# navigator8972/vae_assoc

Hardware: AMD Instinct MI355X
Metric: paired-samples/sec (img+jnt assoc-VAE train step) (higher is better)
Workload: dtype bf16

## Files before the change

__graft_entry__.py:

```python
import os
import subprocess
import sys

ROOT = os.path.dirname(os.path.abspath(__file__))
CSRC = os.path.join(ROOT, "vae_assoc_amd", "csrc")
LIB = os.path.join(ROOT, "vae_assoc_amd", "libavae.so")
SOURCES = ["avae_kernels.hip", "avae_comm.hip", "avae_retrieve.hip", "avae_latent_stats.hip", "avae_aggpost.hip", "avae_gmm.hip", "avae_embed.hip", "avae_host.hip"]


FLAGS = ["--offload-arch=gfx950", "-O3", "-std=c++17", "-fPIC", "-shared", "-Wno-unused-result"]


def _source_hash():
    import hashlib
    h = hashlib.sha256(" ".join(FLAGS).encode())
    for path in sorted(os.path.join(CSRC, f) for f in os.listdir(CSRC)) + [os.path.join(ROOT, "include", "avae.h")]:
        h.update(os.path.basename(path).encode())
        with open(path, "rb") as f:
            h.update(f.read())
    return h.hexdigest()


def _stale(want):
    if not os.path.exists(LIB) or not os.path.exists(LIB + ".hash"):
        return True
    with open(LIB + ".hash") as f:
        return f.read().strip() != want


def build(force=False):
    import fcntl
    want = _source_hash()
    try:
        lock = open(LIB + ".lock", "w")
    except OSError:
        lock = None
        if force or _stale(want):
            raise
    if lock is not None:
        fcntl.flock(lock, fcntl.LOCK_EX)
        try:
            if force or _stale(want):
                hipcc = os.environ.get("HIPCC", "/opt/rocm/bin/hipcc")
                if not os.path.exists(hipcc):
                    hipcc = "hipcc"
                tmp = "%s.tmp.%d" % (LIB, os.getpid())
                cmd = [hipcc] + FLAGS + [os.path.join(CSRC, s) for s in SOURCES] + ["-o", tmp]
                subprocess.run(cmd, check=True, cwd=ROOT)
                os.replace(tmp, LIB)
                with open(LIB + ".hash", "w") as f:
                    f.write(want + "\n")
        finally:
            fcntl.flock(lock, fcntl.LOCK_UN)
            lock.close()
    if ROOT not in sys.path:
        sys.path.insert(0, ROOT)
    import vae_assoc_amd
    from vae_assoc_amd import _capi
    _capi.lib()


def smoke():
    if ROOT not in sys.path:
        sys.path.insert(0, ROOT)
    build()
    import numpy as np
    import torch
    from oracle import vae_assoc_oracle as O
    from vae_assoc_amd.vae_assoc import AssocVariationalAutoEncoder

    assert torch.cuda.is_available(), "smoke() needs the MI355X"
    img = dict(scope='image', hidden_conv=False, n_hidden_recog_1=96, n_hidden_recog_2=80,
               n_hidden_gener_1=96, n_hidden_gener_2=80, n_input=784, n_z=20)
    jnt = dict(scope='joint', hidden_conv=False, n_hidden_recog_1=72, n_hidden_recog_2=40,
               n_hidden_gener_1=72, n_hidden_gener_2=40, n_input=147, n_z=20)
    archs, B = [img, jnt], 48
    rng = np.random.default_rng(7)
    X = [rng.random((B, 784)).astype(np.float32), rng.standard_normal((B, 147)).astype(np.float32)]
    eps = rng.standard_normal((B, 20)).astype(np.float32)
    for dtype, tol in (("fp32", 2e-5), ("bf16", 2e-3)):
        model = AssocVariationalAutoEncoder(archs, binary=[True, False], transfer_fct="relu", weights=[50, 1],
                                            assoc_lambda=8.0, learning_rate=1e-3, batch_size=B,
                                            compute_dtype=dtype, device=0, seed=3)
        ref = O.OracleAssocVAE(archs, binary=[True, False], transfer_fct="relu", weights=[50, 1], assoc_lambda=8.0,
                               learning_rate=1e-3, batch_size=B, params_flat=model.get_params().astype(np.float64))
        c_hip = model.partial_fit(X, eps)
        c_ref = ref.partial_fit(X, eps)
        rel = abs(c_hip - c_ref) / abs(c_ref)
        assert rel < tol, "smoke: %s cost %.6f vs oracle %.6f (rel %.2e)" % (dtype, c_hip, c_ref, rel)
        dp = np.abs(model.get_params() - ref.get_params()).max()
        assert dp < 2.5e-3, "smoke: %s params drifted %.3e after one Adam step" % (dtype, dp)
        print("smoke %s: cost %.5f (oracle %.5f, rel %.2e), max|dtheta| %.2e" % (dtype, c_hip, c_ref, rel, dp))


if __name__ == "__main__":
    build(force="--force" in sys.argv)
    if "--smoke" in sys.argv:
        smoke()
```

vae_assoc_amd/csrc/avae_device.h:

```cpp
#pragma once
#include <hip/hip_runtime.h>
#include <math.h>
#include <stdint.h>
#include "../../include/avae.h"

namespace avae {

constexpr int kMaxMod = 4;
constexpr int kThreads = 256;
constexpr int kTileBytesK = 128;
constexpr int kRowAlign = 256;
constexpr int kLatentRows = 16;
constexpr int kAdamRows = 16;
constexpr int kCostHist = 4096;
constexpr int kSumsqThreads = 256;
constexpr int kSumsqMaxBlocks = 256;
constexpr int kSumsqQuads = 8;
inline int sumsq_blocks(long long p_int) {
    const long long quads = p_int / 4, per_block = (long long)kSumsqThreads * kSumsqQuads;
    const long long g = (quads + per_block - 1) / per_block;
    return (int)(g < 1 ? 1 : g > kSumsqMaxBlocks ? kSumsqMaxBlocks : g);
}
inline int sumsq_chain(long long p_int) {
    const long long quads = p_int / 4, per_pass = (long long)kSumsqThreads * sumsq_blocks(p_int);
    return (int)((quads + per_pass - 1) / per_pass);
}

enum Kind : int {
    K_FWD_HIDDEN = 0,
    K_FWD_HEAD = 1,
    K_FWD_OUT_LOSS = 2,
    K_FWD_OUT_STORE = 3,
    K_DGRAD_HIDDEN = 4,
    K_DGRAD_LATENT = 5,
    K_WGRAD = 6,
    K_DGRAD_F32 = 10,
    K_LATENT = 7,
    K_COST = 8,
    K_SERVE_Z = 11,
};

struct WorkItem {
    int kind;
    int M, N, K;
    int lda, ldb;
    int tiles_m, tiles_n;
    int act;
    int ld0, ld1, ldx;
    int nz;
    int binary;
    int ksplit, kchunk;
    int bias_row;
    int bias_ep;
    int kin;
    int tile_off, tile_cnt;
    int slot_base;
    int n_slots;
    int n_mod;
    int bump_step;
    float scale;
    float lambda;
    float inv_bg;
    const void* A;
    const void* B;
    void* out0;
    void* out1;
    void* out2;
    const void* aux0;
    const void* aux1;
    const void* aux2;
    float* partial;
    const float* eps;
    float wts[kMaxMod];
    const void* tail_w;
    void* tail_out;
    const void* tail_aux;
    int tail_mode;
    int tail_n;
    int tail_ldw, tail_ldo, tail_ldx;
    int tail_act;
    int tail_kt;
    int conv;
    const unsigned char* present;
    int present_ld;
};

struct ConvA {
    const void* src;
    const void* consts;
    int M, K;
    int OHW, OW, IH, IW, Cin;
    int k, so, d, pad;
    int src_sb, src_sp;
    int ones;
    unsigned mg_ohw, mg_ow, mg_k, mg_cin;
};
constexpr int kMaxConvA = 12;
constexpr int kMaxItemsPerLaunch = 12;
constexpr int kMaxPf = 4;
struct LaunchArgs {
    int n_items;
    int grid_x;
    int sched;
    int n_pf;
    const void* pf_ptr[4];
    int pf_lines[4];
    const ConvA* conv_tab;
    WorkItem items[kMaxItemsPerLaunch];
};

struct TnItem {
    const void* A;
    const void* B;
    float* out;
    int M, N, K;
    int lda, ldb, ld0;
    int tiles_m, tiles_n;
    int ksplit, kchunk;
    int bias_row;
    int tile_off, tile_cnt;
    int conv;
    void* W; void* Wt;
    int ldw, ldt;
};
constexpr int kMaxTnItems = 32;
constexpr int kTnPieces = 8;
struct TnPiece { unsigned short item, tile_off, cum_end, pad; };
struct DevState;
struct TnLaunchArgs {
    int n_items;
    int grid_x;
    int xcd_group;
    int sched;
    int adam;
    long long d_theta, d_m, d_v;
    float beta1, beta2, eps;
    const DevState* st;
    const ConvA* conv_tab;
    int xcd_pieces;
    TnPiece pieces[8][kTnPieces];
    TnItem items[kMaxTnItems];
};
static_assert(sizeof(TnLaunchArgs) <= 4096, "kernel arguments are passed by value: 4 KiB");

struct DevState {
    long long step;
    float last_cost;
    float lr_t;
    float cost_hist[kCostHist];
};

struct ClipState {
    float max_norm;
    int skip_nonfinite;
    long long n_skipped;
    float partial[kSumsqMaxBlocks];
    float norm_hist[kCostHist];
};

struct EmaState {
    float decay;
    int warmup;
    int pad[30];
};
static_assert(sizeof(EmaState) == 128, "the average is line-aligned behind its settings");

struct HyperEntry { float kl, lambda, lr, pad; };
constexpr int kHyperSets = 16;
struct SchedState {
    avae_schedule sched[3];
    float lambda0, lr0;
    HyperEntry tab[kHyperSets];
    float hist[kCostHist][3];
};

__host__ __device__ inline float schedule_value(const avae_schedule& s, long long t) {
#pragma clang fp contract(off)
    long long u = t - 1;
    if (u < 0) u = 0;
    if (s.kind == AVAE_SCHED_PIECEWISE) {
        if (s.period > 0) u %= s.period;
        const int last = s.n_knots - 1;
        if (u <= s.knot_step[0]) return s.knot_value[0];
        if (u >= s.knot_step[last]) return s.knot_value[last];
        int i = 0;
        while (i + 1 < last && u >= s.knot_step[i + 1]) ++i;
        const double v0 = (double)s.knot_value[i], v1 = (double)s.knot_value[i + 1];
        const double f = (double)(u - s.knot_step[i]) / (double)(s.knot_step[i + 1] - s.knot_step[i]);
        return (float)(v0 + (v1 - v0) * f);
    }
    if (s.kind == AVAE_SCHED_EXP) {
        const double e = s.staircase ? (double)(u / s.decay_steps) : (double)u / (double)s.decay_steps;
        return (float)pow((double)s.decay_rate, e);
    }
    return 1.0f;
}

struct AdamItem {
    float* theta;
    float* m;
    float* v;
    const float* g;
    void* W;
    void* Wt;
    int rows, cols;
    int ld, ldt;
    int tiles_r, tiles_c, tile_base;
    int ldw;
    void* Wadj; void* Wf;
    int ldadj, ldf, adj_k, adj_cin;
};

constexpr int kMaxAdamItems = 80;
struct AdamArgs {
    const AdamItem* items;
    int n_items;
    int base[kMaxAdamItems];
    int mode;
    int book;
    float lr, beta1, beta2, eps;
    DevState* st;
    const float* cost_src;
    ClipState* clip;
    int n_partial;
    const EmaState* ema;
    float* avg;
    const float* theta0;
};

struct PrepSeg {
    const float* src; int src_ld;
    int rows, cols;
    float* dst32; int ld32;
    void* dstc; int ldc;
    int tiles_r, tiles_c, tile_base;
    const float* src_in; int in_ld;
    unsigned drop_thr;
    float drop_value, noise_std;
};
struct PrepArgs {
    PrepSeg seg[kMaxMod];
    int n_seg;
    int total_tiles;
    const float* eps_src;
    float* eps_dst;
    int eps_rows, nz, eps_blocks, eps_ld;
    int row_offset;
    unsigned long long seed;
    const DevState* st;
    unsigned long long stream_salt;
    int n_steps, blocks_per_step;
    long long set_stride;
    const unsigned char* pres_src;
    unsigned char* pres_dst;
    int pres_ld;
    int noisy;
    SchedState* sched;
};

struct ReduceSeg { float* dst; const float* src; int n, parts; long long stride; int block_base;
                   int dst_ld;
                   int colsum;
                   int perm_k, perm_cin, perm_cout, perm_ldga, perm_ld; };
constexpr int kMaxReduceSegs = 40;
struct ReduceArgs { ReduceSeg seg[kMaxReduceSegs]; int n_seg; };

struct ConvGeom {
    int B, IH, IW, Cin, OH, OW, k, so, d, pad;
    int src_sb, src_sp;
    int ones;
};
struct GatherSeg {
    ConvGeom g;
    const void* src;
    void* P; int ldp;
    int tiles_r, tiles_c, tile_base;
    int cl, rpt;
};
struct GatherArgs { GatherSeg seg[kMaxMod]; int n_seg; };
struct Col2imSeg {
    ConvGeom g;
    const float* dP; int lddp;
    const void* yprev; int ldy;
    int act;
    void* dA; int lda;
    const float* g0; int nz;
    const void* bias; int bias_ld;
    int tiles_r, tiles_c, tile_base;
    int cl, rpt;
};
struct Col2imArgs { Col2imSeg seg[kMaxMod]; int n_seg; };

constexpr int kThinIn = 4096, kThinOut = 1024, kThinF = 1024;
constexpr int kThinSplit = 4;
struct ThinSeg {
    ConvGeom g;
    const void* X;
// ... 21 lines not shown
void launch_wadj(int compute_dtype, const WadjArgs& a, int n_blocks, hipStream_t s);
struct GpermSeg { const float* Gadj; float* G; int ldga, ld, k, Cin, Cout, block_base; };
struct GpermArgs { GpermSeg seg[2 * kMaxMod]; int n_seg; };
void launch_gperm(const GpermArgs& a, int n_blocks, hipStream_t s);
struct RowsumSeg { const void* src; float* part; int ld, rows, cols, cols4, cpow, n_blocks, block_base; };
struct RowsumArgs { RowsumSeg seg[2 * kMaxMod]; int n_seg; };
void launch_rowsum(int compute_dtype, const RowsumArgs& a, int n_blocks, hipStream_t s);

struct ServeSlot {
    const float* z;
    float* out[kMaxMod];
    int rows;
    int pad;
};
struct ServeArgs {
    ServeSlot* slot;
    int n_mod, nz, bucket;
    void* Z[kMaxMod]; int ldz[kMaxMod];
    int blocks_per_mod;
};
void launch_serve(int compute_dtype, const ServeArgs& a, const ServeSlot& call, int n_blocks, hipStream_t s);
struct ServeInMod { const void* w; void* out; int n, ldw, ldo, kt, act, slices; };
struct ServeInArgs {
    ServeSlot call;
    ServeSlot* slot;
    int n_mod, nz, bucket, tiles_m;
    ServeInMod mod[kMaxMod];
};
void launch_serve_in(int compute_dtype, const ServeInArgs& a, int grid_x, hipStream_t s);

void launch_gather(int compute_dtype, const GatherArgs& a, int n_blocks, hipStream_t s);
void launch_col2im(int compute_dtype, const Col2imArgs& a, int n_blocks, hipStream_t s);

constexpr int kScoreRows = kThreads / 64;
struct ScoreLatentArgs {
    const float* mulv[kMaxMod];
    void* Z[kMaxMod]; int ldz[kMaxMod];
    const float* eps; int ld_eps;
    float* out; int k;
    int rows, nz, n_mod;
    int src;
    const unsigned char* present;
};
void launch_score_latent(int compute_dtype, const ScoreLatentArgs& a, hipStream_t s);
struct ScoreRowsArgs {
    const float* xhat; int ld32;
    const float* x; long long ldx;
    float* out; int k;
    int rows, n_in, binary, col;
    int cost;
    int n_mod, n_pair;
    float w[kMaxMod]; float lambda;
    const unsigned char* present; int pa, pb; unsigned absent_bits;
};
void launch_score_rows(const ScoreRowsArgs& a, hipStream_t s);

struct IwLatentArgs {
    const float* mulv;
    const float* eps;
    float* z32;
    void* Z[kMaxMod]; int ldz[kMaxMod]; int n_zdst;
    float* r;
    int rows, kc, k0, K, nz;
    long long row0;
    unsigned long long seed; unsigned draw;
    const unsigned char* present; int pres_ld;
};
void launch_iw_latent(int compute_dtype, const IwLatentArgs& a, hipStream_t s);
struct IwRowsArgs {
    const float* xhat[kMaxMod]; int ldh[kMaxMod];
    const float* x[kMaxMod]; long long ldx[kMaxMod];
    int n_in[kMaxMod], binary[kMaxMod];
    float* ell;
    int n_dec, kc, n_mod;
    const unsigned char* present;
};
void launch_iw_rows(const IwRowsArgs& a, hipStream_t s);
struct IwReduceArgs {
    const float* ell; const float* r;
    float* state;
    float* out; int width;
    int rows, kc, src, n_mod;
    int first, last;
    float log_k;
    const unsigned char* present;
};
void launch_iw_reduce(const IwReduceArgs& a, hipStream_t s);

struct ImputeFuseArgs {
    const float* mulv[kMaxMod];
    unsigned mods;
    const unsigned char* present;
    float* fused;
    float* mu; float* lv;
    float* z32;
    void* Z[kMaxMod]; int ldz[kMaxMod]; int n_zdst;
    int rows, nz, n_mod;
};
void launch_impute_fuse(int compute_dtype, const ImputeFuseArgs& a, hipStream_t s);
struct ImputeAccumArgs {
    const float* xhat[kMaxMod]; int ldh[kMaxMod];
    float* mean[kMaxMod]; float* var[kMaxMod];
    int n_in[kMaxMod];
    int tile0[kMaxMod + 1];
    int col0[kMaxMod];
    float* state; int ld_state;
    int rows, kc, k0, K, n_mod;
};
void launch_impute_accum(const ImputeAccumArgs& a, hipStream_t s);

constexpr int kMaxWorld = 8;
constexpr int kIpcThreads = 256;
struct IpcArgs {
    float* g;
    long long off, granules;
    long long cost_idx;
    int world, rank, wire_bf16, blocks;
    unsigned char* peer[kMaxWorld];
    long long off_flag1, off_flag2;
    long long off_cost;
    long long off_seq;
    long long off_err;
    long long off_slots, slot_stride, off_res;
    unsigned long long timeout_ticks;
};
void launch_ipc_allreduce(const IpcArgs& a, hipStream_t s);
void launch_wire_pack(const float* g, void* wire, long long n, hipStream_t s);
void launch_wire_unpack(float* g, const void* wire, long long n, hipStream_t s);

struct LaunchEvents { hipEvent_t start, stop; };
extern thread_local LaunchEvents t_launch_events;

constexpr int kStampLaunches = 32, kStampBlocks = 1024, kStampWords = 8;

int tile_lds_bytes(int tile_cfg, bool two_c_tiles);
void launch_grouped(int compute_dtype, int tile_cfg, const LaunchArgs& args, int grid_x, int grid_y, int lds_bytes,
                    DevState* st, hipStream_t s, unsigned long long* stamps = nullptr, int launch_id = 0);
void launch_grouped_tn(int compute_dtype, int tile_cfg, const TnLaunchArgs& args, int grid_x, int grid_y, int lds_bytes,
                       DevState* st, hipStream_t s, unsigned long long* stamps = nullptr, int launch_id = 0);
void launch_adam(int compute_dtype, const AdamArgs& a, int n_blocks, hipStream_t s);
void launch_grad_sumsq(const float* g, long long p_int, float* partial, hipStream_t s);
void launch_prep(int compute_dtype, const PrepArgs& a, hipStream_t s);
const void* prep_kernel(int compute_dtype, bool masked, bool noisy, bool sched);
void launch_fill(void* base, int elem_bytes, unsigned bits, long long start, long long stride, int count, hipStream_t s);
void launch_sums(const ReduceArgs& a, int n_blocks, hipStream_t s);
int small_head_lds_bytes();
void launch_small_latb(int compute_dtype, int act, const LaunchArgs& args, int grid_x, int grid_y, int lds_bytes, DevState* st, hipStream_t s,
                       unsigned long long* stamps, int launch_id);
void launch_small_head(int compute_dtype, int act, const LaunchArgs& args, int grid_x, int grid_y, int lds_bytes, hipStream_t s,
                       unsigned long long* stamps, int launch_id);
void launch_small_tn(int compute_dtype, const TnLaunchArgs& args, int grid_x, int grid_y, hipStream_t s, unsigned long long* stamps, int launch_id);
void launch_small_loss(int compute_dtype, const LaunchArgs& args, int grid_x, int grid_y, int lds_bytes, hipStream_t s, unsigned long long* stamps, int launch_id);
void launch_small(int compute_dtype, const LaunchArgs& args, int grid_x, int grid_y, int lds_bytes, hipStream_t s, unsigned long long* stamps, int launch_id);
void launch_reduce(const ReduceArgs& a, int n_blocks, hipStream_t s);
void launch_chain2(int compute_dtype, const LaunchArgs& args, int grid_x, int grid_y, int lds_bytes, unsigned* counters, unsigned* err, hipStream_t s);

}
```

vae_assoc_amd/csrc/avae_host.hip:

```cpp
#include "avae_device.h"
#include "avae_complete.h"
#include "avae_retrieve.h"
#include "avae_latent_stats.h"
#include "avae_gmm.h"
#include "avae_embed.h"
#include "avae_aggpost.h"
#include "../../include/avae.h"

#include <dlfcn.h>
#include <sched.h>
#include <unistd.h>

#include <algorithm>
#include <cctype>
#include <cstddef>
#include <cmath>
#include <cstdio>
#include <cstdlib>
#include <cstring>
#include <functional>
#include <map>
#include <mutex>
#include <stdexcept>
#include <string>
#include <vector>

using namespace avae;

namespace {

thread_local std::string g_create_error;

struct Err : std::runtime_error { using std::runtime_error::runtime_error; };

#define HIP_OK(expr)                                                                             \
    do {                                                                                         \
        hipError_t e_ = (expr);                                                                  \
        if (e_ != hipSuccess)                                                                    \
            throw Err(std::string(#expr) + ": " + hipGetErrorString(e_) + " (" __FILE__ ":" +    \
                      std::to_string(__LINE__) + ")");                                           \
    } while (0)

struct DeviceGuard {
    int prev = -1, want = -1;
    explicit DeviceGuard(int dev) : want(dev) {
        if (hipGetDevice(&prev) != hipSuccess) prev = -1;
        if (prev != want) HIP_OK(hipSetDevice(want));
    }
    ~DeviceGuard() { if (prev >= 0 && prev != want) (void)hipSetDevice(prev); }
    DeviceGuard(const DeviceGuard&) = delete;
    DeviceGuard& operator=(const DeviceGuard&) = delete;
};

#define LAUNCH_OK(what)                                                                          \
    do {                                                                                         \
        hipError_t e_ = hipGetLastError();                                                       \
        if (e_ != hipSuccess) throw Err(std::string("launch of ") + (what) + ": " + hipGetErrorString(e_)); \
    } while (0)

constexpr unsigned long long kTrainSalt = 0x7261696eull;
static_assert(kHyperSets == 16, "one schedule table entry per staging set");
constexpr int kMultiSteps = 16;
constexpr int kMultiSizes[2] = {16, 4};

inline size_t rup(size_t x, size_t a) { return (x + a - 1) / a * a; }

struct Bump {
    size_t off = 0;
    size_t take(size_t bytes) { size_t o = off; off = rup(off + bytes, 256); return o; }
};

struct Dense {
    int in = 0, out = 0;
    int ld = 0;
    int ldw = 0;
    int ldt = 0;
    size_t master = 0;
    size_t W = 0, Wt = 0;
    bool head = false;
};

constexpr int kRowsumBlocks = 256;

struct Act {
    int width = 0;
    int rows = 0;
    int ld = 0;
    size_t rm = 0;
    bool ones = false;
};

struct ConvStage {
    ConvGeom g{};
    Dense d;
    bool bias = false;
    int act = AVAE_ACT_IDENTITY;
    int flat = 0;
    Act P;
    Act Y;
    Act dY;
    size_t dP = 0;
    int lddp = 0;
    int ksplit = 1, kchunk = 0;
    size_t part = 0;
    bool adj = false;
    Act Padj;
    size_t Wadj = 0;
    int ldadj = 0;
    size_t Wf = 0;
    int ldf = 0;
    size_t T = 0;
    int ldT = 0;
    size_t Gadj = 0;
    int ldga = 0, aksplit = 1, akchunk = 0;
    size_t apart = 0;
    size_t rs_part = 0;
    int rs_cols4 = 0;
    bool impl = false;
    bool impl_w = false;
    bool impl_bwd = false;
    int cin_real = 0;
    bool dense_map = false;
    bool thin = false;
    size_t thin_part = 0;
    int thin_blocks = 0, thin_kp = 0;
};

struct Mod {
    int n_in = 0, L = 0;
    std::vector<int> hs;
    std::vector<Dense> enc, dec;
    Dense head, outl;
    Act X0, Z, dH, dO;
    std::vector<Act> E, D, dE, dD;
    size_t X32 = 0, mulv = 0, g0 = 0, out32 = 0;
    int ld32 = 0;
    bool conv = false;
    std::vector<ConvStage> cenc, cdec;
};

struct Launch {
    std::string name;
    int type = 0;
    int cfg = 0, first = 0, count = 0, blocks = 0, lds = 0;
    int lean_act = 0;
    int grid_x = 1, grid_y = 1;
    bool tn = false;
    LaunchArgs args{};
    TnLaunchArgs targs{};
    GatherArgs ga{};
    Col2imArgs ca{};
    ReduceArgs ra{};
    ThinArgs ta{};
    WadjArgs wa{};
    GpermArgs gp{};
    RowsumArgs rs{};
};

struct TimingRec { hipEvent_t a, b; int launch_name; };

struct StepGraph {
    hipGraphExec_t exec = nullptr;
    hipGraph_t graph = nullptr;
    hipGraphNode_t prep = nullptr;
    void release() {
        if (exec) (void)hipGraphExecDestroy(exec);
        if (graph) (void)hipGraphDestroy(graph);
        *this = StepGraph();
    }
};

struct StepPlan {
    std::vector<Launch> fwd;
    StepGraph full, multi[2], eval;
    void release() { full.release(); multi[0].release(); multi[1].release(); eval.release(); }
};

struct DevBuf {
    void* p = nullptr;
    size_t bytes = 0;
    DevBuf() = default;
    DevBuf(const DevBuf&) = delete;
    DevBuf& operator=(const DevBuf&) = delete;
    ~DevBuf() { if (p) (void)hipFree(p); }
    void* ensure(size_t n, bool zero = false) {
        if (p && n != bytes) throw Err("internal error: device scratch of " + std::to_string(bytes) + " bytes asked for as " + std::to_string(n));
        if (p) return p;
        void* q = nullptr;
        HIP_OK(hipMalloc(&q, n));
        if (zero && hipMemset(q, 0, n) != hipSuccess) { (void)hipFree(q); throw Err("hipMemset of fresh device scratch failed"); }
        p = q; bytes = n;
        return p;
    }
    template <typename T> T* as() const { return static_cast<T*>(p); }
};

}

struct avae_handle {
    avae_config cfg{};
    std::mutex mu;
    std::string err;
    int es = 2, KU = 64;
    int B = 0, Bp = 0, ldB = 0;
    int nz = 0, M = 0, ld_eps = 0;
    std::vector<Mod> mods;
    size_t P_flat = 0, P_int = 0, P_enc = 0;
    size_t off_theta = 0, off_m = 0, off_v = 0, off_g = 0;
    size_t stage_lo = 0, stage_bytes = 0;
    size_t off_eps = 0, off_partial = 0, off_state = 0, off_items = 0, off_adam = 0, off_inf = 0, off_stamps = 0, off_latent = 0;
    int n_partial = 0;
    size_t ws_bytes = 0;
    unsigned char* ws = nullptr;
    bool own_ws = false;
    hipStream_t cap_stream = nullptr;

    std::vector<WorkItem> items;
    std::vector<Launch> bwd;
    std::vector<Launch> wgrad;
    std::vector<Launch> wgrad_adam;
    int n_buckets = 1;
    int bwd_split = 0;
    std::vector<Launch> wgrad_b[2];
    struct Range { size_t off, count; };
    std::vector<Range> ranges_b[2];
    int adam_first_b[2] = {0, 0}, adam_count_b[2] = {0, 0}, adam_blocks_b[2] = {0, 0};
    std::vector<AdamItem> adam_items_b;
    size_t off_adam_b = 0;
    void* comm = nullptr;
    int comm_world = 1, comm_rank = 0;
    bool comm_on = false;
    size_t off_wire = 0;
    unsigned char* ipc_block = nullptr;
    size_t ipc_bytes = 0;
    unsigned char* ipc_peer[kMaxWorld] = {nullptr, nullptr, nullptr, nullptr, nullptr, nullptr, nullptr, nullptr};
    bool ipc_opened[kMaxWorld] = {false, false, false, false, false, false, false, false};
    bool ipc_attached = false;
    IpcArgs ipc_args{};
    hipStream_t comm_stream = nullptr;
    hipEvent_t ev_grad[2] = {nullptr, nullptr}, ev_red[2] = {nullptr, nullptr};
    std::vector<StepGraph> g_dp[2];
    StepGraph g_dpm[2];
    bool dp_graph_failed = false;
    Launch cost_only;
    std::vector<AdamItem> adam_items;
    int adam_blocks = 0;
    struct Inf { std::vector<WorkItem> items; std::vector<Launch> launches; int rows = -1; size_t dev_off = 0; };
    std::vector<Inf> inf_enc, inf_dec;
    struct Serve { int bucket = 0; std::vector<WorkItem> items; std::vector<Launch> launches; hipGraphExec_t graph = nullptr; ServeArgs in;
                   Launch in_launch; bool fused_in = false;
                   ServeInArgs in_lean; int in_lean_grid = 0; bool lean_in = false; };
    std::vector<Serve> serve;
    size_t off_slot = 0;
    DevBuf iw_buf;
    DevBuf imp_buf;
    DevBuf row_pres;
    DevBuf topk_buf;
    DevBuf stats_buf;
    DevBuf agg_buf;
    DevBuf gmm_buf;
    DevBuf embed_buf;
    size_t off_chain = 0;
    size_t off_consts = 0, off_conv_tab = 0;
    std::vector<ConvA> conv_tab;

    StepPlan plain, masked;
    DevBuf pres_buf;
    size_t pres_set = 0;

    avae_corruption corr{};
    unsigned drop_thr[kMaxMod] = {};

    bool clip_on = false;
    DevBuf clip_buf;
    long long clip_steps = 0;

    bool sched_on = false;
    DevBuf sched_buf;
    long long sched_steps = 0;

    bool ema_on = false, averaged = false;
    float ema_decay = 0.0f;
    int ema_warmup = 0;
    DevBuf ema_buf;

    struct Complete { bool built = false; std::vector<WorkItem> items; std::vector<Launch> fwd, bwd; CompleteArgs args{};
                      StepGraph g[3]; DevBuf buf; };
    Complete cmpl;

    hipStream_t last_stream = nullptr;
    bool has_last_stream = false;
    hipEvent_t ev_switch = nullptr;
    unsigned draw_id = 0;
    bool timing = false;
    bool debug_sync = false;
    bool plan_dump = false;
    std::vector<std::string> tnames;
    std::vector<TimingRec> trecs;

    template <typename T> T* at(size_t off) const { return reinterpret_cast<T*>(ws + off); }
    DevState* state() const { return at<DevState>(off_state); }
    float* grad() const { return at<float>(off_g); }
    float* ema_avg() const { return reinterpret_cast<float*>(ema_buf.as<unsigned char>() + sizeof(EmaState)); }
};

namespace {

inline int spread_ld(int ld, int KU, int es) {
    static const bool off = std::getenv("AVAE_NO_LD_SPREAD") != nullptr;
    return (!off && ((size_t)ld * es) % 512 == 0) ? ld + KU : ld;
}

Act make_act(Bump& b, int width, bool ones, int rows, int KU, int es, int ld = 0) {
    Act a;
    a.width = width;
    a.rows = rows;
    a.ones = ones;
    a.ld = ld > 0 ? ld : spread_ld((int)rup(width + 1, KU), KU, es);
    a.rm = b.take(rup(rows, kRowAlign) * (size_t)a.ld * es);
    return a;
}

Dense make_dense(Bump& b, size_t& pint, int in, int out, int KU, int es, bool head) {
    Dense d;
    d.in = in; d.out = out; d.head = head;
    d.ld = (int)rup(out, 32);
    d.ldw = spread_ld((int)rup(out, KU), KU, es);
    d.ldt = spread_ld((int)rup(in + 1, KU), KU, es);
    d.master = pint;
    pint += (size_t)(in + 1) * d.ld;
    d.W = b.take(rup(in + 1, kRowAlign) * (size_t)d.ldw * es);
    d.Wt = b.take(rup(out, kRowAlign) * (size_t)d.ldt * es);
    return d;
}

void check_config(const avae_config& c) {
    if (c.abi_version != AVAE_ABI_VERSION) throw Err("avae_config.abi_version mismatch");
    if (c.n_modalities < 1 || c.n_modalities > AVAE_MAX_MODALITIES) throw Err("n_modalities out of range");
    if (c.n_z < 1 || c.n_z > 64) throw Err("n_z must be in [1,64] (the fused head/latent epilogue holds 2*n_z columns in one tile)");
    if (c.batch_size < 1) throw Err("batch_size must be positive");
    if (c.compute_dtype != AVAE_F32 && c.compute_dtype != AVAE_BF16) throw Err("compute_dtype must be AVAE_F32 or AVAE_BF16");
    if (c.activation < AVAE_ACT_IDENTITY || c.activation > AVAE_ACT_TANH) throw Err("unknown activation");
    if (c.comm_buckets != 0 && c.comm_buckets != 1 && c.comm_buckets != 2) throw Err("comm_buckets must be 0, 1 or 2");
    if (c.wire_dtype != AVAE_F32 && c.wire_dtype != AVAE_BF16) throw Err("wire_dtype must be AVAE_F32 or AVAE_BF16");
    if (c.use_comm < AVAE_COMM_NONE || c.use_comm > AVAE_COMM_IPC) throw Err("use_comm must be AVAE_COMM_NONE, AVAE_COMM_RCCL or AVAE_COMM_IPC");
    for (int m = 0; m < c.n_modalities; ++m) {
        const avae_modality& mo = c.mod[m];
        if (mo.n_input < 1) throw Err("n_input must be positive");
        if (mo.hidden_conv) {
            if (mo.n_input != 784) throw Err("hidden_conv needs n_input = 784 (28x28 images)");
            if (!mo.binary) throw Err("hidden_conv needs a binary modality (the reference's non-binary conv decoder is shape-broken, vae_assoc.py:299)");
            if (mo.n_hidden_layers != 2 || mo.conv_gener[0] < 2 || mo.conv_gener[1] < 1) throw Err("hidden_conv needs n_hidden_recog_1/2 and n_hidden_gener_1 (>=2) / n_hidden_gener_2");
        }
        if (mo.n_hidden_layers < 1 || mo.n_hidden_layers > AVAE_MAX_HIDDEN) throw Err("n_hidden_layers out of range");
        for (int k = 0; k < mo.n_hidden_layers; ++k)
            if (mo.n_hidden[k] < 1) throw Err("hidden width must be positive");
    }
}

inline bool thin_fast(const ConvGeom& g) { return thin_fast_geometry(g) && !std::getenv("AVAE_NO_THIN_FAST"); }
inline int thin_split(const ConvGeom& g, int mode) {
    if (!thin_fast(g)) return kThinSplit;
    int sp[3] = {1, 4, 1};
    if (const char* e = std::getenv("AVAE_THIN_FAST_SPLIT")) std::sscanf(e, "%d,%d,%d", &sp[0], &sp[1], &sp[2]);
    const int v = sp[mode];
    return v == 1 || v == 2 || v == 4 ? v : 1;
}

void plan_memory(avae_handle* h) {
    const avae_config& c = h->cfg;
    h->es = c.compute_dtype == AVAE_BF16 ? 2 : 4;
    h->KU = kTileBytesK / h->es;
    h->B = c.batch_size;
    h->Bp = (int)rup(h->B, kRowAlign);
    h->ldB = (int)rup(h->B, h->KU);
    h->nz = c.n_z;
    h->ld_eps = (int)rup(c.n_z, 4);
    h->M = c.n_modalities;
    const int KU = h->KU, es = h->es, Bp = h->Bp, ldB = h->ldB, nz = h->nz, B = h->B;
    Bump b;
    size_t pint = 0, pflat = 0;
    h->mods.clear();
    std::vector<Act> stage_x0(h->M);
    std::vector<size_t> stage_x32(h->M);
    h->stage_lo = b.off;
    for (int m = 0; m < h->M; ++m) {
        const avae_modality& mo = c.mod[m];
        stage_x0[m] = make_act(b, mo.n_input, mo.hidden_conv == 0, B, KU, es);
        stage_x32[m] = b.take((size_t)B * rup(mo.n_input, 8) * 4);
    }
    h->off_eps = b.take((size_t)B * h->ld_eps * 4);
    h->stage_bytes = b.off - h->stage_lo;
    b.take(h->stage_bytes * (kMultiSteps - 1));
    for (int m = 0; m < h->M; ++m) {
        const avae_modality& mo = c.mod[m];
        Mod md;
        md.n_in = mo.n_input;
        md.L = mo.n_hidden_layers;
        md.hs.assign(mo.n_hidden, mo.n_hidden + md.L);
        md.conv = mo.hidden_conv != 0;
        auto act_B = [&](int width, bool ones) { return make_act(b, width, ones, B, KU, es); };
        if (!md.conv) {
            int prev = md.n_in;
            for (int k = 0; k < md.L; ++k) { md.enc.push_back(make_dense(b, pint, prev, md.hs[k], KU, es, false)); pflat += (size_t)(prev + 1) * md.hs[k]; prev = md.hs[k]; }
            md.head = make_dense(b, pint, prev, 2 * nz, KU, es, true);
            pflat += (size_t)(prev + 1) * 2 * nz;
            prev = nz;
            for (int k = 0; k < md.L; ++k) { md.dec.push_back(make_dense(b, pint, prev, md.hs[k], KU, es, false)); pflat += (size_t)(prev + 1) * md.hs[k]; prev = md.hs[k]; }
            md.outl = make_dense(b, pint, prev, md.n_in, KU, es, false);
            pflat += (size_t)(prev + 1) * md.n_in;
            md.X0 = stage_x0[m];
            for (int k = 0; k < md.L; ++k) md.E.push_back(act_B(md.hs[k], true));
            md.Z = act_B(nz, true);
            for (int k = 0; k < md.L; ++k) md.D.push_back(act_B(md.hs[k], true));
// ... 1342 lines not shown
        a.m = h->at<float>(h->off_m) + d.master;
        a.v = h->at<float>(h->off_v) + d.master;
        a.g = h->grad() + d.master;
        a.W = h->at<void>(d.W); a.Wt = h->at<void>(d.Wt);
        a.rows = d.in + 1; a.cols = d.out; a.ld = d.ld; a.ldw = d.ldw; a.ldt = d.ldt;
        a.tiles_r = (a.rows + kAdamRows - 1) / kAdamRows; a.tiles_c = (a.cols + 63) / 64; a.tile_base = base;
        base += a.tiles_r * a.tiles_c;
        h->adam_items.push_back(a);
    };
    for (const Mod& md : h->mods) {
        if (md.conv) {
            for (const std::vector<ConvStage>* side : {&md.cenc, &md.cdec})
                for (const ConvStage& st : *side) {
                    add(st.d);
                    if ((st.adj && !std::getenv("AVAE_NO_WADJ_FOLD")) || st.impl_bwd) {
                        AdamItem& a = h->adam_items.back();
                        a.Wadj = h->at<void>(st.Wadj); a.ldadj = st.ldadj; a.adj_k = st.g.k; a.adj_cin = st.g.Cin;
                        if (st.adj) { a.Wf = h->at<void>(st.Wf); a.ldf = st.ldf; }
                    }
                }
            continue;
        }
        for (const Dense& d : md.enc) add(d);
        add(md.head);
        for (const Dense& d : md.dec) add(d);
        add(md.outl);
    }
    h->adam_blocks = base;
    h->adam_items_b.clear();
    for (int bk = 0; bk < 2; ++bk) {
        h->adam_first_b[bk] = (int)h->adam_items_b.size();
        int tb = 0;
        size_t i = 0;
        for (const Mod& md : h->mods) {
            const size_t n_enc = md.conv ? md.cenc.size() : (size_t)md.L + 1, n_all = md.conv ? md.cenc.size() + md.cdec.size() : 2 * (size_t)md.L + 2;
            for (size_t k = 0; k < n_all; ++k) {
                const int which = h->n_buckets == 1 ? 0 : (k < n_enc ? 1 : 0);
                if (which == bk) {
                    AdamItem a = h->adam_items[i + k];
                    a.tile_base = tb; tb += a.tiles_r * a.tiles_c;
                    h->adam_items_b.push_back(a);
                }
            }
            i += n_all;
        }
        h->adam_count_b[bk] = (int)h->adam_items_b.size() - h->adam_first_b[bk];
        h->adam_blocks_b[bk] = tb;
    }
}

void build_inference(avae_handle* h, int m, bool enc, int rows) {
    avae_handle::Inf& inf = enc ? h->inf_enc[m] : h->inf_dec[m];
    if (inf.rows == rows) return;
    inf.items.clear(); inf.launches.clear();
    Builder bd(h, inf.items, rows, false);
    Mod& md = h->mods[m];
    int slot = 0;
    auto one = [&](const WorkItem& w, const std::string& name) {
        inf.items.push_back(w);
        inf.launches.push_back(finish_launch(h, inf.items, (int)inf.items.size() - 1, 1, name, &slot));
    };
    auto gather1 = [&](const ConvStage& st, const void* src, const std::string& name) {
        Launch L;
        L.name = name; L.type = 1;
        GatherSeg g = bd.gather_seg(st, src);
        g.tile_base = 0;
        L.ga.seg[0] = g; L.ga.n_seg = 1;
        L.blocks = g.tiles_r * g.tiles_c;
        inf.launches.push_back(L);
    };
    if (enc && md.conv) {
        for (int i = 0; i < 3; ++i) {
            gather1(md.cenc[i], i == 0 ? h->at<void>(md.X0.rm) : h->at<void>(md.cenc[i - 1].Y.rm), "inf_conv_im2col");
            one(bd.conv_fwd(md.cenc[i]), "inf_conv_enc");
        }
        gather1(md.cenc[3], h->at<void>(md.cenc[2].Y.rm), "inf_conv_im2col");
        one(bd.fwd_head(md, true), "inf_head");
    } else if (enc) {
        for (int k = 0; k < md.L; ++k) one(bd.fwd_hidden(k == 0 ? md.X0 : md.E[k - 1], md.enc[k], md.E[k]), "inf_enc");
        one(bd.fwd_head(md, true), "inf_head");
    } else if (md.conv) {
        for (int i = 0; i < 4; ++i) {
            if (md.cdec[i].dense_map) {
                Launch L;
                L.name = "inf_conv_dec_direct"; L.type = 4;
                L.ta.mode = 0;
                ThinSeg t = bd.thin_seg(md.cdec[i], md.cdec[i - 1]);
                t.block_base = 0;
                L.ta.seg[0] = t; L.ta.n_seg = 1;
                L.blocks = rows * t.split;
                inf.launches.push_back(L);
                continue;
            }
            gather1(md.cdec[i], i == 0 ? h->at<void>(md.Z.rm) : h->at<void>(md.cdec[i - 1].Y.rm), "inf_conv_im2col");
            one(bd.conv_fwd(md.cdec[i]), "inf_conv_dec");
        }
        if (!md.cdec[3].dense_map) gather1(md.cdec[4], h->at<void>(md.cdec[3].Y.rm), "inf_conv_im2col");
        one(bd.fwd_out(md, m, false), "inf_out");
    } else {
        for (int k = 0; k < md.L; ++k) one(bd.fwd_hidden(k == 0 ? md.Z : md.D[k - 1], md.dec[k], md.D[k]), "inf_dec");
        one(bd.fwd_out(md, m, false), "inf_out");
    }
    inf.rows = rows;
}

int tname_id(avae_handle* h, const std::string& n) {
    for (size_t i = 0; i < h->tnames.size(); ++i) if (h->tnames[i] == n) return (int)i;
    h->tnames.push_back(n);
    return (int)h->tnames.size() - 1;
}

struct Timed {
    avae_handle* h; hipStream_t s; bool on; hipEvent_t a = nullptr, b = nullptr; int id = 0;
    Timed(avae_handle* h_, hipStream_t s_, const std::string& name) : h(h_), s(s_), on(h_->timing && h_->trecs.size() < 200000) {
        if (!on) return;
        id = tname_id(h, name);
        HIP_OK(hipEventCreate(&a)); HIP_OK(hipEventCreate(&b));
        t_launch_events = LaunchEvents{a, b};
    }
    ~Timed() {
        if (!on) return;
        if (t_launch_events.start) {
            t_launch_events = LaunchEvents{nullptr, nullptr};
            (void)hipEventRecord(a, s); (void)hipEventRecord(b, s);
        }
        h->trecs.push_back(TimingRec{a, b, id});
    }
};

template <typename F> void timed_launch(avae_handle* h, hipStream_t s, const char* name, F&& launch) {
    Timed t(h, s, name);
    launch();
    LAUNCH_OK(name);
}

Launch relocated(const avae_handle* h, const Launch& L0, int j, const HyperEntry* hyper = nullptr) {
    Launch L = L0;
    const unsigned char* lo = h->ws + h->stage_lo;
    const unsigned char* hi = lo + h->stage_bytes;
    const size_t delta = (size_t)j * h->stage_bytes;
    auto fix = [&](auto& ptr) {
        const unsigned char* q = reinterpret_cast<const unsigned char*>(ptr);
        if (q >= lo && q < hi) ptr = reinterpret_cast<std::remove_reference_t<decltype(ptr)>>(const_cast<unsigned char*>(q) + delta);
    };
    for (int i = 0; i < L.args.n_items && L.type == 0; ++i) {
        WorkItem& w = L.args.items[i];
        fix(w.A); fix(w.B); fix(w.out0); fix(w.out1); fix(w.out2); fix(w.aux0); fix(w.aux1); fix(w.aux2); fix(w.eps);
        fix(w.tail_w); fix(w.tail_out); fix(w.tail_aux);
        if (w.present) w.present += (size_t)j * h->pres_set;
        if (hyper && (w.kind == K_LATENT || (w.kind == K_COST && w.bump_step))) w.tail_w = hyper + j;
    }
    for (int i = 0; i < L.targs.n_items && L.type == 0; ++i) { TnItem& t = L.targs.items[i]; fix(t.A); fix(t.B); fix(t.out); }
    for (int i = 0; i < L.ga.n_seg && L.type == 1; ++i) fix(L.ga.seg[i].src);
    return L;
}

void dump_launch(const Launch& L) {
    std::fprintf(stderr, "[avae] launch %s type=%d cfg=%d items=%d blocks=%d\n", L.name.c_str(), L.type, L.cfg, L.count, L.blocks);
    for (int i = 0; i < L.args.n_items && L.type == 0; ++i)
        std::fprintf(stderr, "        item kind=%d M=%d N=%d K=%d lda=%d ldb=%d tiles=%dx%d\n", L.args.items[i].kind, L.args.items[i].M,
                     L.args.items[i].N, L.args.items[i].K, L.args.items[i].lda, L.args.items[i].ldb, L.args.items[i].tiles_m, L.args.items[i].tiles_n);
    for (int i = 0; i < L.ga.n_seg && L.type == 1; ++i)
        std::fprintf(stderr, "        gather B=%d IH=%d Cin=%d OH=%d k=%d so=%d d=%d pad=%d sb=%d sp=%d ones=%d ldp=%d tiles=%dx%d\n", L.ga.seg[i].g.B, L.ga.seg[i].g.IH,
                     L.ga.seg[i].g.Cin, L.ga.seg[i].g.OH, L.ga.seg[i].g.k, L.ga.seg[i].g.so, L.ga.seg[i].g.d, L.ga.seg[i].g.pad, L.ga.seg[i].g.src_sb, L.ga.seg[i].g.src_sp,
                     L.ga.seg[i].g.ones, L.ga.seg[i].ldp, L.ga.seg[i].tiles_r, L.ga.seg[i].tiles_c);
    for (int i = 0; i < L.ca.n_seg && L.type == 2; ++i)
        std::fprintf(stderr, "        col2im B=%d IH=%d Cin=%d OH=%d k=%d lddp=%d lda=%d g0=%p tiles=%dx%d\n", L.ca.seg[i].g.B, L.ca.seg[i].g.IH, L.ca.seg[i].g.Cin,
                     L.ca.seg[i].g.OH, L.ca.seg[i].g.k, L.ca.seg[i].lddp, L.ca.seg[i].lda, (const void*)L.ca.seg[i].g0, L.ca.seg[i].tiles_r, L.ca.seg[i].tiles_c);
}

void run_launch(avae_handle* h, const Launch& L, hipStream_t s, unsigned long long* stamps, int stamp) {
    Timed t(h, s, L.name);
    if (L.type == 1) launch_gather(h->cfg.compute_dtype, L.ga, L.blocks, s);
    else if (L.type == 2) launch_col2im(h->cfg.compute_dtype, L.ca, L.blocks, s);
    else if (L.type == 3) launch_reduce(L.ra, L.blocks, s);
    else if (L.type == 4) launch_thin(h->cfg.compute_dtype, L.ta, L.blocks, s);
    else if (L.type == 5) launch_colsum(L.ra, L.blocks, s);
    else if (L.type == 6) launch_wadj(h->cfg.compute_dtype, L.wa, L.blocks, s);
    else if (L.type == 7) launch_gperm(L.gp, L.blocks, s);
    else if (L.type == 8) launch_rowsum(h->cfg.compute_dtype, L.rs, L.blocks, s);
    else if (L.type == 9) launch_sums(L.ra, L.blocks, s);
    else if (L.cfg == 13) launch_chain2(h->cfg.compute_dtype, L.args, L.grid_x, L.grid_y, L.lds, h->at<unsigned>(h->off_chain), h->at<unsigned>(h->off_chain) + kMaxMod * 64, s);
    else if (L.cfg == 11) launch_small_head(h->cfg.compute_dtype, L.lean_act, L.args, L.grid_x, L.grid_y, L.lds, s, stamps, stamp);
    else if (L.cfg == 10) launch_small_latb(h->cfg.compute_dtype, L.lean_act, L.args, L.grid_x, L.grid_y, L.lds, h->state(), s, stamps, stamp);
    else if (L.cfg == 9) launch_small_loss(h->cfg.compute_dtype, L.args, L.grid_x, L.grid_y, L.lds, s, stamps, stamp);
    else if (L.cfg == 7) launch_small(h->cfg.compute_dtype, L.args, L.grid_x, L.grid_y, L.lds, s, stamps, stamp);
    else if (L.tn && L.cfg == 12) launch_small_tn(h->cfg.compute_dtype, L.targs, L.grid_x, L.grid_y, s, stamps, stamp);
    else if (L.tn) launch_grouped_tn(h->cfg.compute_dtype, L.cfg, L.targs, L.grid_x, L.grid_y, L.lds, h->state(), s, stamps, stamp);
    else launch_grouped(h->cfg.compute_dtype, L.cfg, L.args, L.grid_x, L.grid_y, L.lds, h->state(), s, stamps, stamp);
    LAUNCH_OK(L.name);
    if (h->debug_sync) {
        dump_launch(L);
        std::fflush(stderr);
        HIP_OK(hipStreamSynchronize(s));
    }
}

bool has_hyper_item(const Launch& L) {
    for (int i = 0; i < L.args.n_items && L.type == 0; ++i)
        if (L.args.items[i].kind == K_LATENT || (L.args.items[i].kind == K_COST && L.args.items[i].bump_step)) return true;
    return false;
}

void run_set(avae_handle* h, const std::vector<Launch>& ls, size_t lo, size_t hi, int j, hipStream_t s, int stamp_base = -1, bool train = false) {
    unsigned long long* stamps = nullptr;
#ifdef AVAE_STAMPS
    if (stamp_base >= 0) stamps = h->at<unsigned long long>(h->off_stamps);
#endif
    const HyperEntry* hyper = nullptr;
    if (train && h->sched_on) {
        if (!h->sched_buf.p) throw Err("internal error: a schedule is on without its device state");
        if (j < 0 || j >= kHyperSets) throw Err("internal error: staging set outside the schedule table");
        hyper = h->sched_buf.as<SchedState>()->tab;
    }
    for (size_t i = lo; i < hi && i < ls.size(); ++i) {
        const int k = stamp_base + (int)(i - lo);
        if (j == 0 && !(hyper && has_hyper_item(ls[i]))) run_launch(h, ls[i], s, stamps, k);
        else run_launch(h, relocated(h, ls[i], j, hyper), s, stamps, k);
    }
}

void run_launches(avae_handle* h, const std::vector<Launch>& ls, hipStream_t s) { run_set(h, ls, 0, ls.size(), 0, s); }

void run_adam(avae_handle* h, int mode, hipStream_t s, int bucket = -1, bool from_avg = false) {
    AdamArgs a;
    std::memset(&a, 0, sizeof(a));
    int blocks = h->adam_blocks;
    if (bucket < 0) {
        a.items = h->at<AdamItem>(h->off_adam);
        a.n_items = (int)h->adam_items.size();
        if (a.n_items > kMaxAdamItems) throw Err("internal error: too many Adam items");
        for (int i = 0; i < a.n_items; ++i) a.base[i] = h->adam_items[i].tile_base;
    } else {
        a.items = h->at<AdamItem>(h->off_adam_b) + h->adam_first_b[bucket];
        a.n_items = h->adam_count_b[bucket];
        for (int i = 0; i < a.n_items; ++i) a.base[i] = h->adam_items_b[h->adam_first_b[bucket] + i].tile_base;
        blocks = h->adam_blocks_b[bucket];
        if (blocks == 0) return;
    }
    a.book = (bucket <= 0) ? 1 : 0;
    a.mode = mode;
    a.lr = h->cfg.learning_rate; a.beta1 = h->cfg.beta1; a.beta2 = h->cfg.beta2; a.eps = h->cfg.adam_eps;
    a.st = h->state();
    a.cost_src = h->grad() + h->P_int;
    a.clip = (mode == 0 && h->clip_on) ? h->clip_buf.as<ClipState>() : nullptr;
    a.n_partial = sumsq_blocks((long long)h->P_int);
    if (mode == 0 ? h->ema_on : from_avg) {
        if (!h->ema_buf.p) throw Err("internal error: averaging is on without its device state");
        a.ema = h->ema_buf.as<EmaState>(); a.avg = h->ema_avg(); a.theta0 = h->at<float>(h->off_theta);
    }
    Timed t(h, s, mode == 0 ? (bucket < 0 ? "adam" : bucket == 0 ? "adam_dec" : "adam_enc") : "shadow_refresh");
    launch_adam(h->cfg.compute_dtype, a, blocks, s);
    LAUNCH_OK(mode == 0 ? "adam" : "shadow_refresh");
}

void run_grad_sumsq(avae_handle* h, hipStream_t s) {
    ClipState* cs = h->clip_buf.as<ClipState>();
    if (!cs) throw Err("internal error: clipping is on without its device state");
    timed_launch(h, s, "grad_sumsq", [&] { launch_grad_sumsq(h->grad(), (long long)h->P_int, cs->partial, s); });
}

struct PrepIn { const float* const* in = nullptr; const int32_t* in_ld = nullptr; bool corrupt = false; };

PrepArgs new_prep(const avae_handle* h, unsigned long long salt, int row0 = 0) {
    PrepArgs a;
    std::memset(&a, 0, sizeof(a));
    a.row_offset = h->cfg.row_offset + row0; a.seed = h->cfg.seed; a.st = h->state(); a.stream_salt = salt;
    return a;
}

int fill_prep_seg(const avae_handle* h, PrepSeg& g, const float* src, int src_ld, int rows, int cols, const Act& dst, float* dst32,
                  int ld32, int tile_base) {
    g.src = src; g.src_ld = src_ld; g.rows = rows; g.cols = cols;
    g.dst32 = dst32; g.ld32 = ld32;
    g.dstc = h->at<void>(dst.rm); g.ldc = dst.ld;
    g.tiles_r = (rows + 63) / 64; g.tiles_c = (cols + 63) / 64; g.tile_base = tile_base;
    return g.tiles_r * g.tiles_c;
}

void fill_prep_eps(const avae_handle* h, PrepArgs& a, const float* eps, int rows) {
    a.eps_src = eps; a.eps_dst = h->at<float>(h->off_eps); a.eps_rows = rows; a.nz = h->nz; a.eps_ld = h->ld_eps;
    a.eps_blocks = (rows * ((h->nz + 3) / 4) + kThreads - 1) / kThreads;
}

PrepArgs make_prep_batch(avae_handle* h, const float* const* x, const int32_t* x_ld, const float* eps, int rows,
                         unsigned long long salt, int n_steps = 1, const uint8_t* present = nullptr, const PrepIn& pin = PrepIn()) {
    PrepArgs a = new_prep(h, salt);
    int base = 0;
    for (int m = 0; m < h->M; ++m) {
        const Mod& md = h->mods[m];
        PrepSeg& g = a.seg[m];
        base += fill_prep_seg(h, g, x[m], (x_ld && x_ld[m] > 0) ? x_ld[m] : md.n_in, rows, md.n_in, md.X0, h->at<float>(md.X32), md.ld32, base);
        if (pin.in && pin.in[m]) {
            g.src_in = pin.in[m]; g.in_ld = (pin.in_ld && pin.in_ld[m] > 0) ? pin.in_ld[m] : md.n_in;
            a.noisy = 1;
        } else if (pin.corrupt && (h->drop_thr[m] != 0u || h->corr.noise_std[m] > 0.0f)) {
            g.drop_thr = h->drop_thr[m]; g.drop_value = h->corr.drop_value[m]; g.noise_std = h->corr.noise_std[m];
            a.noisy = 1;
        }
    }
    a.n_seg = h->M; a.total_tiles = base;
    fill_prep_eps(h, a, eps, rows);
    a.n_steps = n_steps; a.blocks_per_step = a.total_tiles + a.eps_blocks; a.set_stride = (long long)h->stage_bytes;
    if (present) { a.pres_src = present; a.pres_dst = h->pres_buf.as<unsigned char>(); a.pres_ld = h->M; }
    if (h->sched_on && salt == kTrainSalt) a.sched = h->sched_buf.as<SchedState>();
    return a;
}

void run_prep_batch(avae_handle* h, const float* const* x, const int32_t* x_ld, const float* eps, int rows,
                    unsigned long long salt, hipStream_t s, const uint8_t* present = nullptr, int n_steps = 1, const PrepIn& pin = PrepIn()) {
    const PrepArgs a = make_prep_batch(h, x, x_ld, eps, rows, salt, n_steps, present, pin);
    timed_launch(h, s, "prep", [&] { launch_prep(h->cfg.compute_dtype, a, s); });
}

struct PrepOne {
    const float* src; int src_ld, rows, cols;
    const Act& dst;
    int row0;
    PrepOne(const float* src_, int src_ld_, int rows_, int cols_, const Act& dst_, int row0_ = 0)
        : src(src_), src_ld(src_ld_), rows(rows_), cols(cols_), dst(dst_), row0(row0_) {}
    float* dst32 = nullptr; int ld32 = 0;
    bool eps = false;
    const float* eps_src = nullptr;
    unsigned long long salt = 0;
    PrepOne& with_eps(const float* e, unsigned long long salt_ = 0) { eps = true; eps_src = e; salt = salt_; return *this; }
    const unsigned char* pres_src = nullptr; unsigned char* pres_dst = nullptr; int pres_ld = 0;
};

void run_prep_single(avae_handle* h, const PrepOne& p, hipStream_t s) {
    PrepArgs a = new_prep(h, p.salt, p.row0);
    if (p.pres_src) { a.pres_src = p.pres_src; a.pres_dst = p.pres_dst; a.pres_ld = p.pres_ld; }
    if (p.src || p.pres_src) {
        a.n_seg = 1;
        a.total_tiles = fill_prep_seg(h, a.seg[0], p.src, p.src_ld, p.rows, p.cols, p.dst, p.dst32, p.ld32, 0);
    }
    if (p.eps) fill_prep_eps(h, a, p.eps_src, p.rows);
    launch_prep(h->cfg.compute_dtype, a, s);
    LAUNCH_OK("prep");
}

StepGraph capture(avae_handle* h, const std::function<void(hipStream_t)>& body, bool with_prep = false) {
    StepGraph sg;
    const bool tsave = h->timing;
    h->timing = false;
    HIP_OK(hipStreamBeginCapture(h->cap_stream, hipStreamCaptureModeThreadLocal));
    try { body(h->cap_stream); }
    catch (...) { (void)hipStreamEndCapture(h->cap_stream, &sg.graph); sg.release(); h->timing = tsave; throw; }
    h->timing = tsave;
    HIP_OK(hipStreamEndCapture(h->cap_stream, &sg.graph));
    try {
        if (with_prep) {
            size_t n_root = 0;
            HIP_OK(hipGraphGetRootNodes(sg.graph, nullptr, &n_root));
            if (n_root != 1) throw Err("internal error: the captured step is not a chain");
            HIP_OK(hipGraphGetRootNodes(sg.graph, &sg.prep, &n_root));
            hipGraphNodeType ty;
            HIP_OK(hipGraphNodeGetType(sg.prep, &ty));
            if (ty != hipGraphNodeTypeKernel) throw Err("internal error: the captured step does not start with the staging kernel");
        }
        HIP_OK(hipGraphInstantiate(&sg.exec, sg.graph, nullptr, nullptr, 0));
        if (!with_prep) { HIP_OK(hipGraphDestroy(sg.graph)); sg.graph = nullptr; }
    } catch (...) { sg.release(); throw; }
    return sg;
}

void patch_prep(avae_handle* h, const StepGraph& sg, const float* const* x, const int32_t* x_ld, const float* eps,
                int n_steps, const uint8_t* present, const PrepIn& pin) {
    PrepArgs a = make_prep_batch(h, x, x_ld, eps, h->B, kTrainSalt, n_steps, present, pin);
    void* kp[1] = {&a};
    hipKernelNodeParams np;
    std::memset(&np, 0, sizeof(np));
    np.func = const_cast<void*>(prep_kernel(h->cfg.compute_dtype, present != nullptr, a.noisy != 0, a.sched != nullptr));
    np.gridDim = dim3((a.total_tiles + a.eps_blocks) * n_steps); np.blockDim = dim3(kThreads);
    np.sharedMemBytes = 0; np.kernelParams = kp; np.extra = nullptr;
    HIP_OK(hipGraphExecKernelNodeSetParams(sg.exec, sg.prep, &np));
}

void fill_ones(avae_handle* h, const Act& a, hipStream_t s) {
    if (!a.ones) return;
    const unsigned bits = h->es == 2 ? 0x3F80u : 0x3F800000u;
    launch_fill(h->at<void>(a.rm), h->es, bits, a.width, a.ld, h->B, s);
    LAUNCH_OK("fill");
}

void step_body(avae_handle* h, const std::vector<Launch>& fwd, hipStream_t s, int j, int stamp_base = -1) {
    auto sb = [&](size_t k) { return stamp_base < 0 ? -1 : stamp_base + (int)k; };
    run_set(h, fwd, 0, fwd.size(), j, s, stamp_base, true);
    run_set(h, h->bwd, 0, h->bwd.size(), j, s, sb(fwd.size()), true);
    if (!h->wgrad_adam.empty() && !h->clip_on && !h->ema_on) {
        run_set(h, h->wgrad_adam, 0, h->wgrad_adam.size(), j, s, sb(fwd.size() + h->bwd.size()), true);
        return;
    }
    run_set(h, h->wgrad, 0, h->wgrad.size(), j, s, sb(fwd.size() + h->bwd.size()), true);
    if (h->clip_on) run_grad_sumsq(h, s);
    run_adam(h, 0, s);
}

void capture_steps(avae_handle* h, StepPlan& p, const uint8_t* present) {
    std::vector<const float*> x0(h->M, h->at<float>(h->mods[0].X32));
    try {
        p.full = capture(h, [&](hipStream_t cs) {
            run_prep_batch(h, x0.data(), nullptr, nullptr, h->B, kTrainSalt, cs, present);
            step_body(h, p.fwd, cs, 0, 0);
        }, true);
        for (int gi = 0; gi < 2; ++gi) p.multi[gi] = capture(h, [&](hipStream_t cs) {
            run_prep_batch(h, x0.data(), nullptr, nullptr, h->B, kTrainSalt, cs, present, kMultiSizes[gi]);
            for (int j = 0; j < kMultiSizes[gi]; ++j) step_body(h, p.fwd, cs, j);
        }, true);
    } catch (...) { p.full.release(); p.multi[0].release(); p.multi[1].release(); throw; }
}

void capture_plan(avae_handle* h, StepPlan& p, const uint8_t* present) {
    try {
        capture_steps(h, p, present);
        p.eval = capture(h, [&](hipStream_t cs) { run_launches(h, p.fwd, cs); run_launch(h, h->cost_only, cs, nullptr, -1); });
    } catch (...) { p.release(); throw; }
}

void init_device(avae_handle* h) {
    hipStream_t s = h->cap_stream;
    HIP_OK(hipMemsetAsync(h->ws, 0, h->ws_bytes, s));
    for (const Mod& md : h->mods) {
        for (int j = 0; j < kMultiSteps; ++j) {
            Act x = md.X0;
            x.rm += (size_t)j * h->stage_bytes;
            fill_ones(h, x, s);
        }
        for (const Act& a : md.E) fill_ones(h, a, s);
        fill_ones(h, md.Z, s);
        for (const Act& a : md.D) fill_ones(h, a, s);
        if (md.conv && md.cdec[3].dense_map) fill_ones(h, md.cdec[3].Y, s);
    }
    build_training_plan(h);
    HIP_OK(hipMemcpyAsync(h->at<void>(h->off_adam), h->adam_items.data(), h->adam_items.size() * sizeof(AdamItem), hipMemcpyHostToDevice, s));
    HIP_OK(hipMemcpyAsync(h->at<void>(h->off_adam_b), h->adam_items_b.data(), h->adam_items_b.size() * sizeof(AdamItem), hipMemcpyHostToDevice, s));
    {
        static const unsigned char c32_bf16[32] = {0, 0, 0, 0, 0, 0, 0, 0, 0, 0, 0, 0, 0, 0, 0, 0, 0x80, 0x3F};
        static const unsigned char c32_f32[32] = {0, 0, 0, 0, 0, 0, 0, 0, 0, 0, 0, 0, 0, 0, 0, 0, 0, 0, 0x80, 0x3F};
        HIP_OK(hipMemcpyAsync(h->at<void>(h->off_consts), h->es == 2 ? c32_bf16 : c32_f32, 32, hipMemcpyHostToDevice, s));
        if (!h->conv_tab.empty()) {
            const unsigned char* lo = h->ws + h->stage_lo;
            for (const ConvA& c : h->conv_tab)
                if (reinterpret_cast<const unsigned char*>(c.src) >= lo && reinterpret_cast<const unsigned char*>(c.src) < lo + h->stage_bytes * kMultiSteps)
                    throw Err("internal error: an implicit patch matrix on a staged input (not relocatable per step)");
            HIP_OK(hipMemcpyAsync(h->at<void>(h->off_conv_tab), h->conv_tab.data(), h->conv_tab.size() * sizeof(ConvA), hipMemcpyHostToDevice, s));
        }
    }
    size_t off = h->off_inf;
    h->inf_enc.assign(h->M, avae_handle::Inf());
    h->inf_dec.assign(h->M, avae_handle::Inf());
    for (int m = 0; m < h->M; ++m) {
        h->inf_enc[m].dev_off = off; off += ((size_t)h->mods[m].L + 1) * sizeof(WorkItem);
        h->inf_dec[m].dev_off = off; off += ((size_t)h->mods[m].L + 1) * sizeof(WorkItem);
    }
    HIP_OK(hipStreamSynchronize(s));
    if (h->cfg.use_graph) capture_plan(h, h->plain, nullptr);
}

void comm_check_error(avae_handle* h);

void fetch_cost(avae_handle* h, float* cost_host, bool from_state, hipStream_t s) {
    if (!cost_host) return;
    const void* src = from_state ? (const void*)&h->state()->last_cost : (const void*)(h->grad() + h->P_int);
    HIP_OK(hipMemcpyAsync(cost_host, src, sizeof(float), hipMemcpyDeviceToHost, s));
    HIP_OK(hipStreamSynchronize(s));
    comm_check_error(h);
}

void copy_rows(void* dst, size_t dpitch, const void* src, size_t spitch, size_t width, size_t rows, hipStream_t s) {
    HIP_OK(hipMemcpy2DAsync(dst, dpitch, src, spitch, width, rows, hipMemcpyDeviceToDevice, s));
}

hipStream_t on_stream(avae_handle* h, void* stream) {
    hipStream_t s = reinterpret_cast<hipStream_t>(stream);
    if (h->has_last_stream && s != h->last_stream) {
        if (!h->ev_switch) HIP_OK(hipEventCreateWithFlags(&h->ev_switch, hipEventDisableTiming));
        if (hipEventRecord(h->ev_switch, h->last_stream) == hipSuccess) HIP_OK(hipStreamWaitEvent(s, h->ev_switch, 0));
        else (void)hipGetLastError();
    }
    h->last_stream = s; h->has_last_stream = true;
    return s;
}

void check_schedule(const avae_schedule& c, const std::string& who) {
    auto fail = [&](const std::string& what) { throw Err(who + ": " + what); };
    if (c.kind == AVAE_SCHED_NONE) return;
    if (c.kind == AVAE_SCHED_PIECEWISE) {
        if (c.n_knots < 1 || c.n_knots > AVAE_SCHED_MAX_KNOTS)
            fail("n_knots = " + std::to_string(c.n_knots) + " must be in [1, " + std::to_string(AVAE_SCHED_MAX_KNOTS) + "]");
        if (c.period < 0) fail("period = " + std::to_string((long long)c.period) + " must be >= 0");
        for (int i = 0; i < c.n_knots; ++i) {
            if (i == 0 ? c.knot_step[0] < 0 : c.knot_step[i] <= c.knot_step[i - 1])
                fail("knot_step[" + std::to_string(i) + "] = " + std::to_string((long long)c.knot_step[i]) +
                     (i == 0 ? " must be >= 0" : " must be above knot_step[" + std::to_string(i - 1) + "] (strictly increasing)"));
            if (!(c.knot_value[i] >= 0.0f) || std::isinf(c.knot_value[i]))
                fail("knot_value[" + std::to_string(i) + "] must be finite and >= 0");
        }
        if (c.period > 0 && c.knot_step[c.n_knots - 1] >= c.period)
            fail("knot_step[" + std::to_string(c.n_knots - 1) + "] = " + std::to_string((long long)c.knot_step[c.n_knots - 1]) +
                 " must be below period = " + std::to_string((long long)c.period));
        return;
    }
    if (c.kind == AVAE_SCHED_EXP) {
        if (!(c.decay_rate > 0.0f) || std::isinf(c.decay_rate)) fail("decay_rate must be finite and > 0");
        if (c.decay_steps <= 0) fail("decay_steps = " + std::to_string((long long)c.decay_steps) + " must be > 0");
        if (c.staircase != 0 && c.staircase != 1) fail("staircase must be 0 or 1");
        return;
    }
    fail("kind = " + std::to_string(c.kind) + " is none of AVAE_SCHED_NONE, AVAE_SCHED_PIECEWISE, AVAE_SCHED_EXP");
}

avae_schedule canonical_schedule(const avae_schedule& c) {
    avae_schedule o;
    std::memset(&o, 0, sizeof(o));
    o.kind = c.kind;
    if (c.kind == AVAE_SCHED_PIECEWISE) {
        o.n_knots = c.n_knots; o.period = c.period;
        for (int i = 0; i < c.n_knots; ++i) { o.knot_step[i] = c.knot_step[i]; o.knot_value[i] = c.knot_value[i]; }
    } else if (c.kind == AVAE_SCHED_EXP) {
        o.decay_rate = c.decay_rate; o.staircase = c.staircase; o.decay_steps = c.decay_steps;
    }
    return o;
}

template <typename F> int guarded(avae_handle* h, F&& f) {
    if (!h) return 1;
    std::lock_guard<std::mutex> lk(h->mu);
    try {
        DeviceGuard dg(h->cfg.device);
        f();
        return 0;
    } catch (const std::exception& e) {
        h->err = e.what();
        return 2;
    }
}

void master_to_host(avae_handle* h, size_t off, std::vector<float>& host) {
    host.resize(h->P_int);
    HIP_OK(hipDeviceSynchronize());
    HIP_OK(hipMemcpy(host.data(), h->at<void>(off), h->P_int * 4, hipMemcpyDeviceToHost));
}
void host_to_master(avae_handle* h, size_t off, const std::vector<float>& host) {
    HIP_OK(hipDeviceSynchronize());
    HIP_OK(hipMemcpy(h->at<void>(off), host.data(), h->P_int * 4, hipMemcpyHostToDevice));
}

struct Rccl {
    struct Id { char b[128]; };
    typedef int (*get_id_t)(void*);
    typedef int (*init_rank_t)(void**, int, Id, int);
    typedef int (*all_reduce_t)(const void*, void*, size_t, int, int, void*, hipStream_t);
    typedef int (*destroy_t)(void*);
    typedef const char* (*err_t)(int);
    typedef int (*group_t)();
    void* lib = nullptr;
    get_id_t get_id = nullptr; init_rank_t init_rank = nullptr; all_reduce_t all_reduce = nullptr; destroy_t destroy = nullptr;
    err_t err_str = nullptr; group_t group_start = nullptr, group_end = nullptr;
    static Rccl& get() {
        static Rccl r;
        static std::once_flag once;
        std::call_once(once, [] {
            const char* names[] = {"librccl.so", "librccl.so.1", "/opt/rocm/lib/librccl.so.1", "/opt/rocm/lib/librccl.so"};
            for (const char* n : names) if ((r.lib = dlopen(n, RTLD_NOW | RTLD_NOLOAD))) break;
            for (const char* n : names) { if (r.lib) break; r.lib = dlopen(n, RTLD_NOW | RTLD_LOCAL); }
            if (!r.lib) return;
            r.get_id = (get_id_t)dlsym(r.lib, "ncclGetUniqueId"); r.init_rank = (init_rank_t)dlsym(r.lib, "ncclCommInitRank");
            r.all_reduce = (all_reduce_t)dlsym(r.lib, "ncclAllReduce"); r.destroy = (destroy_t)dlsym(r.lib, "ncclCommDestroy");
            r.err_str = (err_t)dlsym(r.lib, "ncclGetErrorString");
            r.group_start = (group_t)dlsym(r.lib, "ncclGroupStart"); r.group_end = (group_t)dlsym(r.lib, "ncclGroupEnd");
        });
        if (!r.lib || !r.get_id || !r.init_rank || !r.all_reduce || !r.destroy || !r.group_start || !r.group_end)
            throw Err("RCCL is not available (librccl.so could not be loaded): the library-owned gradient all-reduce needs it");
        return r;
    }
};
#define NCCL_OK(expr)                                                                            \
    do {                                                                                         \
        int r_ = (expr);                                                                         \
        if (r_ != 0) throw Err(std::string(#expr) + ": " + (Rccl::get().err_str ? Rccl::get().err_str(r_) : "RCCL error") + " (" + std::to_string(r_) + ")"); \
    } while (0)
constexpr int kNcclFloat32 = 7, kNcclSum = 0;

constexpr int kNcclBfloat16 = 9;
constexpr uint32_t kIpcMagic = 0x41564950u;
struct IpcHandleBytes {
// ... 2132 lines not shown
```

vae_assoc_amd/csrc/avae_kernels.hip:

```cpp
#include "avae_device.h"
#include "avae_complete.h"
#include <hip/hip_ext.h>
#include <stdexcept>
#include "../../include/avae.h"

namespace avae {

typedef __attribute__((ext_vector_type(8))) __bf16 bf16x8;
typedef __attribute__((ext_vector_type(4))) __bf16 bf16x4;
typedef __attribute__((ext_vector_type(4))) float f32x4;
typedef __attribute__((ext_vector_type(4))) unsigned u32x4;


template <typename CT> __device__ __forceinline__ CT to_ct(float v);
template <> __device__ __forceinline__ float to_ct<float>(float v) { return v; }
template <> __device__ __forceinline__ __bf16 to_ct<__bf16>(float v) { return (__bf16)v; }

__device__ __forceinline__ float bf16_bits_to_float(unsigned b) { return __uint_as_float(b << 16); }

template <typename CT> __device__ __forceinline__ void load4(const CT* p, float v[4]);
template <> __device__ __forceinline__ void load4<float>(const float* p, float v[4]) {
    float4 t = *reinterpret_cast<const float4*>(p);
    v[0] = t.x; v[1] = t.y; v[2] = t.z; v[3] = t.w;
}
// ... 1122 lines not shown
                    if (q >= QE) { q -= QE; ++row; }
                }
#pragma unroll
                for (int k = 0; k < HALF; ++k) {
                    if (rws[k] < BM) {
#pragma unroll
                        for (int e = 0; e < 4; ++e) {
                            const int d = 4 * qs[k] + e;
                            if (d < nz) {
                                const float dz = Cs[cs_idx<LDC>(rws[k], d)];
                                Zs[cs_idx<LDC>(rws[k], d)] = dz + gm[k][e];
                                Zs[cs_idx<LDC>(rws[k], nz + d)] = __builtin_fmaf(dz, gf[k][e], gl[k][e]);
                            }
                        }
                    }
                }
            }
        }
        lds_barrier();
        if (ts == 0)
            tile_pass<CT, CT, false, false, BM, BN>(Zs, reinterpret_cast<CT*>(w.out0), w.ld0, (const CT*)nullptr, 8,
                                                    M, 2 * nz, m0, 0, [](float c, float, bool) { return c; });
        if (tail_on) { t_src = Zs; t_cols = 2 * nz; t_one = -1; }
      }
    } break;
    case K_SERVE_Z: {
      if constexpr (TAIL) {
        const int nz = w.nz, rows = w.n_slots;
        float* Zs = Cs + BM * LDC;
        const float* zsrc = reinterpret_cast<const float*>(w.aux0);
        for (int i = tid; i < BM * nz; i += NT) {
            const int r = i / nz, d = i - r * nz;
            Zs[cs_idx<LDC>(r, d)] = m0 + r < rows ? zsrc[(size_t)(m0 + r) * nz + d] : 0.0f;
        }
        if (blockIdx.x == 0 && blockIdx.y == 0 && tid == 0) {
            ServeSlot* sp = reinterpret_cast<ServeSlot*>(w.partial);
            sp->z = zsrc; sp->rows = rows;
            sp->out[0] = reinterpret_cast<float*>(w.out0); sp->out[1] = reinterpret_cast<float*>(w.out1);
            sp->out[2] = reinterpret_cast<float*>(w.out2); sp->out[3] = reinterpret_cast<float*>(const_cast<void*>(w.aux1));
        }
        lds_barrier();
        if (tail_on) { t_src = Zs; t_cols = nz; t_one = nz; }
      }
    } break;
    case K_DGRAD_F32:
    case K_WGRAD: {
        float* G = reinterpret_cast<float*>(w.out0);
        tile_pass<float, float, false, false, BM, BN, NT>(Cs, G, w.ld0, (const float*)nullptr, 4, M, N, m0, n0,
            [](float c, float, bool) { return c; });
    } break;
    default: break;
    }
    if (t_src) tail_product(t_src, t_cols, t_one);
    AVAE_STAMP(4)
    AVAE_STAMP_FLUSH()
    return;
    }
    if constexpr (!TN && (NW == 4 || (NW == 8 && BN == 64))) {
        if (w.kind == K_LATENT) latent_item<NW, MASK>(w, t, red);
        else cost_item<NW>(w, st, red);
        AVAE_STAMP(4)
        AVAE_STAMP_FLUSH()
    }
}

template <typename CT, int KIND, int ACT>
__global__ void __launch_bounds__(kThreads) k_small(const LaunchArgs args, unsigned long long* stamps, int launch_id) {
    constexpr int BM = 32, RING = 4, ES = (int)sizeof(CT), NCH = 2;
    constexpr int kStage = 64 * kTileBytesK;
    unsigned char* smem = avae_dyn_smem;
#ifdef AVAE_STAMPS
    unsigned long long sv[kStampWords] = {0, 0, 0, 0, 0, 0, 0, 0};
#endif
    AVAE_STAMP(0)
    const int part = blockIdx.x & 7, idx = blockIdx.x >> 3;
    const WorkItem w = args.items[blockIdx.y];
    asm volatile("" :: "s"(w.A), "s"(w.B), "s"(w.out0), "s"(w.aux0), "s"(w.lda), "s"(w.ldb), "s"(w.K), "s"(w.ld0), "s"(w.ldx));
    int t;
    {
        const int nt = w.tiles_m * w.tiles_n;
        const int q = nt >> 3, r = nt & 7;
        if (idx >= q + (part < r ? 1 : 0)) return;
        t = (part < r ? part * (q + 1) : r * (q + 1) + (part - r) * q) + idx;
    }
    const int tid = threadIdx.x, lane = tid & 63, wave = __builtin_amdgcn_readfirstlane(tid >> 6);
    const int wr = wave >> 1, wc = wave & 1, fr = lane & 15, fq = lane >> 4;
    const int tm = t / w.tiles_n, tn = t - tm * w.tiles_n;
    const int m0 = tm * BM, n0 = tn * 32;
    const int nk = (w.K * ES) / kTileBytesK;
    typedef const __attribute__((address_space(1))) void* gp_t;
    typedef __attribute__((address_space(3))) void* lp_t;
    const int prow = wave * 8 + (lane >> 3), lc = ((lane & 7) ^ ((prow >> 1) & 7)) * 16;
    const unsigned char* srcA = reinterpret_cast<const unsigned char*>(w.A) + (size_t)(m0 + prow) * w.lda * ES + lc;
    const unsigned char* srcB = reinterpret_cast<const unsigned char*>(w.B) + (size_t)(n0 + prow) * w.ldb * ES + lc;
    const int orow = m0 + wr * 16 + fr, ocol = n0 + wc * 16 + 4 * fq;
    typename Quad<CT>::raw yq;
    if constexpr (KIND == 1)
        yq = *reinterpret_cast<const typename Quad<CT>::raw*>(reinterpret_cast<const CT*>(w.aux0) + (size_t)min(orow, w.M - 1) * w.ldx + min(ocol, w.ldx - 4));
#define AVAE_S_DMA(kt, buf)                                                                                             \
    { __builtin_amdgcn_global_load_lds((gp_t)(srcA + (size_t)(kt) * kTileBytesK), (lp_t)(smem + (buf) * kStage + wave * 1024), 16, 0, 0);          \
      __builtin_amdgcn_global_load_lds((gp_t)(srcB + (size_t)(kt) * kTileBytesK), (lp_t)(smem + (buf) * kStage + (4 + wave) * 1024), 16, 0, 0); }
    AVAE_STAMP(1)
    const int npro = nk < RING - 1 ? nk : RING - 1;
    for (int p = 0; p < npro; ++p) AVAE_S_DMA(p, p)
    const int sw0 = (fq ^ (fr >> 1)) * 16;
    const int aoff = (wr * 16 + fr) * kTileBytesK, boff = (32 + wc * 16 + fr) * kTileBytesK;
    f32x4 acc = {0.f, 0.f, 0.f, 0.f};
    int buf = 0;
    for (int kt = 0; kt < nk; ++kt) {
        const int rem = nk - 1 - kt;
        if (rem >= 2) asm volatile("s_waitcnt vmcnt(4)" ::: "memory");
        else if (rem == 1) asm volatile("s_waitcnt vmcnt(2)" ::: "memory");
        else asm volatile("s_waitcnt vmcnt(0)" ::: "memory");
        asm volatile("s_barrier" ::: "memory");
        if (kt == 0) { AVAE_STAMP(2) }
        const unsigned char* Sb = smem + buf * kStage;
        const u32x4 a0 = *reinterpret_cast<const u32x4*>(Sb + aoff + sw0), b0 = *reinterpret_cast<const u32x4*>(Sb + boff + sw0);
        const int fill = buf == 0 ? RING - 1 : buf - 1;
        if (kt + RING - 1 < nk) AVAE_S_DMA(kt + RING - 1, fill)
        const u32x4 a1 = *reinterpret_cast<const u32x4*>(Sb + aoff + (sw0 ^ 64)), b1 = *reinterpret_cast<const u32x4*>(Sb + boff + (sw0 ^ 64));
        mma<CT>(b0, a0, acc);
        mma<CT>(b1, a1, acc);
        buf = buf + 1 == RING ? 0 : buf + 1;
    }
#undef AVAE_S_DMA
    AVAE_STAMP(3)
    if constexpr (KIND == 2) {
        float v[4];
#pragma unroll
        for (int e = 0; e < 4; ++e) v[e] = w.binary ? sigmoidf_(acc[e]) : acc[e];
        if (w.aux2) {
            const ServeSlot* sp = reinterpret_cast<const ServeSlot*>(w.aux2);
            float* dst = sp->out[w.n_mod] + (size_t)orow * w.N + ocol;
            if (orow < sp->rows) {
#pragma unroll
                for (int e = 0; e < 4; ++e) if (ocol + e < w.N) dst[e] = v[e];
            }
        } else if (orow < w.M && ocol < w.N) {
            store_row<float>(reinterpret_cast<float*>(w.out0) + (size_t)orow * w.ld0 + ocol, v, w.N - ocol);
        }
    } else if (orow < w.M && ocol < w.N) {
        float v[4];
#pragma unroll
        for (int e = 0; e < 4; ++e) {
            if constexpr (KIND == 0) v[e] = act_fwd_t<ACT>(acc[e]);
            else v[e] = acc[e] * act_bwd_t<ACT>(quad_elem<CT>(yq, e));
        }
        store_row<CT>(reinterpret_cast<CT*>(w.out0) + (size_t)orow * w.ld0 + ocol, v, w.N - ocol);
    }
    AVAE_STAMP(4)
    AVAE_STAMP_FLUSH()
}

thread_local LaunchEvents t_launch_events = {nullptr, nullptr};

#define AVAE_LAUNCH(kernel, grid, block, lds, stream, ...)                                                   \
    do {                                                                                                     \
        if (t_launch_events.start) {                                                                         \
            hipExtLaunchKernelGGL(kernel, grid, block, lds, stream, t_launch_events.start, t_launch_events.stop, 0, __VA_ARGS__); \
            t_launch_events = LaunchEvents{nullptr, nullptr};                                                \
        } else {                                                                                             \
            hipLaunchKernelGGL(kernel, grid, block, lds, stream, __VA_ARGS__);                               \
        }                                                                                                    \
    } while (0)

template <typename K> static void set_max_lds(K kernel) {
    (void)hipFuncSetAttribute(reinterpret_cast<const void*>(kernel), hipFuncAttributeMaxDynamicSharedMemorySize, 160 * 1024);
}

template <typename CT, bool MASK>
__global__ void __launch_bounds__(kThreads) k_small_loss(const LaunchArgs args, unsigned long long* stamps, int launch_id) {
    constexpr int BM = 32, RING = 4, ES = (int)sizeof(CT);
    constexpr int kStage = 64 * kTileBytesK;
    unsigned char* smem = avae_dyn_smem;
    float* red = reinterpret_cast<float*>(smem + RING * kStage);
#ifdef AVAE_STAMPS
    unsigned long long sv[kStampWords] = {0, 0, 0, 0, 0, 0, 0, 0};
#endif
    AVAE_STAMP(0)
    const int part = blockIdx.x & 7, idx = blockIdx.x >> 3;
    const WorkItem w = args.items[blockIdx.y];
    asm volatile("" :: "s"(w.A), "s"(w.B), "s"(w.out0), "s"(w.aux0), "s"(w.lda), "s"(w.ldb), "s"(w.K), "s"(w.ld0), "s"(w.ldx));
    int t;
    {
        const int nt = w.tiles_m * w.tiles_n;
        const int q = nt >> 3, r = nt & 7;
        if (idx >= q + (part < r ? 1 : 0)) return;
        t = (part < r ? part * (q + 1) : r * (q + 1) + (part - r) * q) + idx;
    }
    if (w.kind == K_LATENT) {
        latent_item<4, MASK>(w, t, red);
        AVAE_STAMP(4)
        AVAE_STAMP_FLUSH()
        return;
    }
    const int tid = threadIdx.x, lane = tid & 63, wave = __builtin_amdgcn_readfirstlane(tid >> 6);
    const int wr = wave >> 1, wc = wave & 1, fr = lane & 15, fq = lane >> 4;
    const int tm = t / w.tiles_n, tn = t - tm * w.tiles_n;
    const int m0 = tm * BM, n0 = tn * 32;
    const int nk = (w.K * ES) / kTileBytesK;
    typedef const __attribute__((address_space(1))) void* gp_t;
    typedef __attribute__((address_space(3))) void* lp_t;
    const int prow = wave * 8 + (lane >> 3), lc = ((lane & 7) ^ ((prow >> 1) & 7)) * 16;
    const unsigned char* srcA = reinterpret_cast<const unsigned char*>(w.A) + (size_t)(m0 + prow) * w.lda * ES + lc;
    const unsigned char* srcB = reinterpret_cast<const unsigned char*>(w.B) + (size_t)(n0 + prow) * w.ldb * ES + lc;
    const int orow = m0 + wr * 16 + fr, ocol = n0 + wc * 16 + 4 * fq;
    const f32x4 xq = *reinterpret_cast<const f32x4*>(reinterpret_cast<const float*>(w.aux0) + (size_t)min(orow, w.M - 1) * w.ldx + min(ocol, w.ldx - 4));
    const bool rpres = !MASK || w.present[(size_t)min(orow, w.M - 1) * w.present_ld] != 0;
#define AVAE_S_DMA(kt, buf)                                                                                             \
    { __builtin_amdgcn_global_load_lds((gp_t)(srcA + (size_t)(kt) * kTileBytesK), (lp_t)(smem + (buf) * kStage + wave * 1024), 16, 0, 0);          \
      __builtin_amdgcn_global_load_lds((gp_t)(srcB + (size_t)(kt) * kTileBytesK), (lp_t)(smem + (buf) * kStage + (4 + wave) * 1024), 16, 0, 0); }
    AVAE_STAMP(1)
    const int npro = nk < RING - 1 ? nk : RING - 1;
    for (int p = 0; p < npro; ++p) AVAE_S_DMA(p, p)
    const int sw0 = (fq ^ (fr >> 1)) * 16;
    const int aoff = (wr * 16 + fr) * kTileBytesK, boff = (32 + wc * 16 + fr) * kTileBytesK;
    f32x4 acc = {0.f, 0.f, 0.f, 0.f};
    int buf = 0;
    for (int kt = 0; kt < nk; ++kt) {
        const int rem = nk - 1 - kt;
        if (rem >= 2) asm volatile("s_waitcnt vmcnt(4)" ::: "memory");
        else if (rem == 1) asm volatile("s_waitcnt vmcnt(2)" ::: "memory");
        else asm volatile("s_waitcnt vmcnt(0)" ::: "memory");
        asm volatile("s_barrier" ::: "memory");
        if (kt == 0) { AVAE_STAMP(2) }
        const unsigned char* Sb = smem + buf * kStage;
        const u32x4 a0 = *reinterpret_cast<const u32x4*>(Sb + aoff + sw0), b0 = *reinterpret_cast<const u32x4*>(Sb + boff + sw0);
        const int fill = buf == 0 ? RING - 1 : buf - 1;
        if (kt + RING - 1 < nk) AVAE_S_DMA(kt + RING - 1, fill)
        const u32x4 a1 = *reinterpret_cast<const u32x4*>(Sb + aoff + (sw0 ^ 64)), b1 = *reinterpret_cast<const u32x4*>(Sb + boff + (sw0 ^ 64));
        mma<CT>(b0, a0, acc);
        mma<CT>(b1, a1, acc);
        buf = buf + 1 == RING ? 0 : buf + 1;
    }
#undef AVAE_S_DMA
    AVAE_STAMP(3)
    const float sc = w.scale;
    float csum = 0.0f, v[4];
#pragma unroll
    for (int e = 0; e < 4; ++e) {
        const bool ok = orow < w.M && ocol + e < w.N && rpres;
        float sl, da;
        if (w.binary) loss_bernoulli(acc[e], xq[e], sc, sl, da);
        else loss_gauss(acc[e], xq[e], sc, sl, da);
        csum += ok ? sl : 0.0f;
        v[e] = ok ? da : 0.0f;
    }
    if (orow < w.M && ocol < w.N) store_row<CT>(reinterpret_cast<CT*>(w.out0) + (size_t)orow * w.ld0 + ocol, v, w.N - ocol);
    const float total = block_sum<4>(csum, red);
    if (tid == 0) w.partial[w.slot_base + t] = total;
    AVAE_STAMP(4)
    AVAE_STAMP_FLUSH()
}
void launch_small_loss(int compute_dtype, const LaunchArgs& args, int grid_x, int grid_y, int lds_bytes, hipStream_t s, unsigned long long* stamps, int launch_id) {
    const dim3 grid(grid_x, grid_y), block(kThreads);
    bool masked = false;
    for (int i = 0; i < args.n_items; ++i) masked = masked || args.items[i].present != nullptr;
    if (masked) {
        if (compute_dtype == AVAE_BF16) AVAE_LAUNCH((k_small_loss<__bf16, true>), grid, block, lds_bytes, s, args, stamps, launch_id);
        else AVAE_LAUNCH((k_small_loss<float, true>), grid, block, lds_bytes, s, args, stamps, launch_id);
    } else if (compute_dtype == AVAE_BF16) AVAE_LAUNCH((k_small_loss<__bf16, false>), grid, block, lds_bytes, s, args, stamps, launch_id);
    else AVAE_LAUNCH((k_small_loss<float, false>), grid, block, lds_bytes, s, args, stamps, launch_id);
}

constexpr int kHeadStage = (32 + 64) * kTileBytesK, kHeadImg = 2 * 32 * kTileBytesK;
int small_head_lds_bytes() { return 4 * kHeadStage + kHeadImg + 64; }

template <typename CT> __device__ __forceinline__ void img_put(unsigned char* img, int row, int d, float v) {
    const int b = d * (int)sizeof(CT), bo = b & 127;
    *reinterpret_cast<CT*>(img + (b >> 7) * (32 * kTileBytesK) + row * kTileBytesK + ((((bo >> 4) ^ ((row >> 1) & 7)) << 4) | (bo & 15))) = to_ct<CT>(v);
}

template <typename CT, int ACT>
__global__ void __launch_bounds__(kThreads) k_small_latb(const LaunchArgs args, DevState* st, unsigned long long* stamps, int launch_id) {
    constexpr int RING = 4, ES = (int)sizeof(CT), TSL = ES == 2 ? 2 : 4;
    unsigned char* smem = avae_dyn_smem;
    unsigned char* img = smem + RING * kHeadStage;
    float* red = reinterpret_cast<float*>(img + kHeadImg);
#ifdef AVAE_STAMPS
    unsigned long long sv[kStampWords] = {0, 0, 0, 0, 0, 0, 0, 0};
#endif
    AVAE_STAMP(0)
    const int part = blockIdx.x & 7, idx = blockIdx.x >> 3;
    const WorkItem w = args.items[blockIdx.y];
    asm volatile("" :: "s"(w.A), "s"(w.B), "s"(w.out0), "s"(w.aux2), "s"(w.lda), "s"(w.ldb), "s"(w.K), "s"(w.ld0), "s"(w.tail_w), "s"(w.tail_out), "s"(w.tail_aux));
    int t;
    {
        const int nt = w.tiles_m * w.tiles_n;
        const int q = nt >> 3, r = nt & 7;
        if (idx >= q + (part < r ? 1 : 0)) return;
        t = (part < r ? part * (q + 1) : r * (q + 1) + (part - r) * q) + idx;
    }
    if (w.kind == K_COST) {
        cost_item<4>(w, st, red);
        AVAE_STAMP(4)
        AVAE_STAMP_FLUSH()
        return;
    }
    const int tid = threadIdx.x, lane = tid & 63, wave = __builtin_amdgcn_readfirstlane(tid >> 6);
    const int wr = wave >> 1, wc = wave & 1, fr = lane & 15, fq = lane >> 4;
    const int tm = t / w.tiles_n, ts = t - tm * w.tiles_n;
    const int m0 = tm * 32;
    const int nk = (w.K * ES) / kTileBytesK, nz = w.nz;
    typedef const __attribute__((address_space(1))) void* gp_t;
    typedef __attribute__((address_space(3))) void* lp_t;
    reinterpret_cast<f32x4*>(img)[tid] = f32x4{0.f, 0.f, 0.f, 0.f};
// ... 122 lines not shown
    const int wr = wave >> 1, wc = wave & 1, fr = lane & 15, fq = lane >> 4;
    const int tm = t / w.tiles_n, ts = t - tm * w.tiles_n;
    const int m0 = tm * 32;
    const int nk = (w.K * ES) / kTileBytesK, nz = w.nz;
    typedef const __attribute__((address_space(1))) void* gp_t;
    typedef __attribute__((address_space(3))) void* lp_t;
    reinterpret_cast<f32x4*>(img)[tid] = f32x4{0.f, 0.f, 0.f, 0.f};
    reinterpret_cast<f32x4*>(img)[tid + kThreads] = f32x4{0.f, 0.f, 0.f, 0.f};
    const int zrow = tid >> 3, zg = tid & 7;
    const f32x4 ev = *reinterpret_cast<const f32x4*>(reinterpret_cast<const float*>(w.aux0) + (size_t)min(m0 + zrow, w.M - 1) * w.ldx + min(4 * zg, w.ldx - 4));
    const int t_i = wave & 1, t_c0 = (2 * ts + (wave >> 1)) * 32, t_sl = 2 * w.tail_kt;
    u32x4 tb[TSL][2];
#pragma unroll
    for (int j = 0; j < 2; ++j) {
        const unsigned char* pw = reinterpret_cast<const unsigned char*>(w.tail_w) + (size_t)min(t_c0 + 16 * j + fr, w.tail_n - 1) * w.tail_ldw * ES + fq * 16;
#pragma unroll
        for (int sl = 0; sl < TSL; ++sl) if (TSL == 2 || sl < t_sl) tb[sl][j] = *reinterpret_cast<const u32x4*>(pw + 64 * sl);
    }
    const int prow = wave * 8 + (lane >> 3), lc = ((lane & 7) ^ ((prow >> 1) & 7)) * 16;
    const unsigned char* srcA = reinterpret_cast<const unsigned char*>(w.A) + (size_t)(m0 + prow) * w.lda * ES + lc;
    const unsigned char* srcB = reinterpret_cast<const unsigned char*>(w.B) + (size_t)prow * w.ldb * ES + lc;
    const size_t b32 = (size_t)32 * w.ldb * ES;
#define AVAE_H_DMA(kt, buf)                                                                                             \
    { __builtin_amdgcn_global_load_lds((gp_t)(srcA + (size_t)(kt) * kTileBytesK), (lp_t)(smem + (buf) * kHeadStage + wave * 1024), 16, 0, 0);       \
      __builtin_amdgcn_global_load_lds((gp_t)(srcB + (size_t)(kt) * kTileBytesK), (lp_t)(smem + (buf) * kHeadStage + (4 + wave) * 1024), 16, 0, 0); \
      __builtin_amdgcn_global_load_lds((gp_t)(srcB + b32 + (size_t)(kt) * kTileBytesK), (lp_t)(smem + (buf) * kHeadStage + (8 + wave) * 1024), 16, 0, 0); }
    AVAE_STAMP(1)
    const int npro = nk < RING - 1 ? nk : RING - 1;
    for (int p = 0; p < npro; ++p) AVAE_H_DMA(p, p)
    const int sw0 = (fq ^ (fr >> 1)) * 16;
    const int aoff = (wr * 16 + fr) * kTileBytesK, boff = (32 + wc * 32 + fr) * kTileBytesK;
    f32x4 acc[2] = {{0.f, 0.f, 0.f, 0.f}, {0.f, 0.f, 0.f, 0.f}};
    int buf = 0;
    for (int kt = 0; kt < nk; ++kt) {
        const int rem = nk - 1 - kt;
        if (rem >= 2) asm volatile("s_waitcnt vmcnt(6)" ::: "memory");
        else if (rem == 1) asm volatile("s_waitcnt vmcnt(3)" ::: "memory");
        else asm volatile("s_waitcnt vmcnt(0)" ::: "memory");
        asm volatile("s_barrier" ::: "memory");
        if (kt == 0) { AVAE_STAMP(2) }
        const unsigned char* Sb = smem + buf * kHeadStage;
        const u32x4 a0 = *reinterpret_cast<const u32x4*>(Sb + aoff + sw0);
        const u32x4 b00 = *reinterpret_cast<const u32x4*>(Sb + boff + sw0), b01 = *reinterpret_cast<const u32x4*>(Sb + boff + 16 * kTileBytesK + sw0);
        const int fill = buf == 0 ? RING - 1 : buf - 1;
        if (kt + RING - 1 < nk) AVAE_H_DMA(kt + RING - 1, fill)
        const u32x4 a1 = *reinterpret_cast<const u32x4*>(Sb + aoff + (sw0 ^ 64));
        const u32x4 b10 = *reinterpret_cast<const u32x4*>(Sb + boff + (sw0 ^ 64)), b11 = *reinterpret_cast<const u32x4*>(Sb + boff + 16 * kTileBytesK + (sw0 ^ 64));
        mma<CT>(b00, a0, acc[0]); mma<CT>(b01, a0, acc[1]);
        mma<CT>(b10, a1, acc[0]); mma<CT>(b11, a1, acc[1]);
        buf = buf + 1 == RING ? 0 : buf + 1;
    }
#undef AVAE_H_DMA
    lds_barrier();
    AVAE_STAMP(3)
    {
        const int orow = m0 + wr * 16 + fr, lrow = wr * 16 + fr;
        float* mulv = reinterpret_cast<float*>(w.out0) + (size_t)orow * w.ld0;
        const bool store = ts == 0 && orow < w.M;
#pragma unroll
        for (int j = 0; j < 2; ++j) {
            const int c0 = wc * 32 + j * 16 + 4 * fq;
            *reinterpret_cast<f32x4*>(MV + lrow * LDM + c0) = acc[j];
            if (store) {
#pragma unroll
                for (int e = 0; e < 4; ++e) if (c0 + e < 2 * nz) mulv[c0 + e] = acc[j][e];
            }
        }
    }
    lds_barrier();
    AVAE_STAMP(5)
    {
        CT* Z = reinterpret_cast<CT*>(w.out1) + (size_t)(m0 + zrow) * w.ld1;
        const bool store = ts == 0 && m0 + zrow < w.M;
#pragma unroll
        for (int e = 0; e < 4; ++e) {
            const int d = 4 * zg + e;
            if (d < nz) {
                const float z = __builtin_fmaf(fexp(0.5f * MV[zrow * LDM + nz + d]), ev[e], MV[zrow * LDM + d]);
                img_put<CT>(img, zrow, d, z);
                if (store) Z[d] = to_ct<CT>(z);
            }
        }
        if (tid < 32) img_put<CT>(img, tid, nz, 1.0f);
    }
    lds_barrier();
    AVAE_STAMP_EP(6)
    {
        const int arow = 16 * t_i + fr;
        f32x4 tacc[1][2] = {{{0.f, 0.f, 0.f, 0.f}, {0.f, 0.f, 0.f, 0.f}}};
#pragma unroll
        for (int sl = 0; sl < TSL; ++sl)
            if (TSL == 2 || sl < t_sl) {
                const u32x4 ta = *reinterpret_cast<const u32x4*>(img + (sl >> 1) * (32 * kTileBytesK) + arow * kTileBytesK + (((fq + 4 * (sl & 1)) ^ ((arow >> 1) & 7)) << 4));
                mma<CT>(tb[sl][0], ta, tacc[0][0]);
                mma<CT>(tb[sl][1], ta, tacc[0][1]);
            }
        regep_store<CT, 1, 2>(tacc, reinterpret_cast<CT*>(w.tail_out), w.tail_ldo, w.M, w.tail_n, m0 + arow, t_c0, lane,
            [&](int, int, int, float v) { return act_fwd_t<ACT>(v); });
    }
    AVAE_STAMP(4)
    AVAE_STAMP_FLUSH()
}
void launch_small_head(int compute_dtype, int act, const LaunchArgs& args, int grid_x, int grid_y, int lds_bytes, hipStream_t s,
                       unsigned long long* stamps, int launch_id) {
    const dim3 grid(grid_x, grid_y), block(kThreads);
#define K_HEAD_B(A) k_small_head<__bf16, A>
#define K_HEAD_F(A) k_small_head<float, A>
    if (compute_dtype == AVAE_BF16) {
        switch (act) {
            case AVAE_ACT_RELU: AVAE_LAUNCH((K_HEAD_B(AVAE_ACT_RELU)), grid, block, lds_bytes, s, args, stamps, launch_id); break;
            case AVAE_ACT_SOFTPLUS: AVAE_LAUNCH((K_HEAD_B(AVAE_ACT_SOFTPLUS)), grid, block, lds_bytes, s, args, stamps, launch_id); break;
            case AVAE_ACT_SIGMOID: AVAE_LAUNCH((K_HEAD_B(AVAE_ACT_SIGMOID)), grid, block, lds_bytes, s, args, stamps, launch_id); break;
            case AVAE_ACT_TANH: AVAE_LAUNCH((K_HEAD_B(AVAE_ACT_TANH)), grid, block, lds_bytes, s, args, stamps, launch_id); break;
            default: AVAE_LAUNCH((K_HEAD_B(AVAE_ACT_IDENTITY)), grid, block, lds_bytes, s, args, stamps, launch_id); break;
        }
    } else {
        switch (act) {
            case AVAE_ACT_RELU: AVAE_LAUNCH((K_HEAD_F(AVAE_ACT_RELU)), grid, block, lds_bytes, s, args, stamps, launch_id); break;
            case AVAE_ACT_SOFTPLUS: AVAE_LAUNCH((K_HEAD_F(AVAE_ACT_SOFTPLUS)), grid, block, lds_bytes, s, args, stamps, launch_id); break;
            case AVAE_ACT_SIGMOID: AVAE_LAUNCH((K_HEAD_F(AVAE_ACT_SIGMOID)), grid, block, lds_bytes, s, args, stamps, launch_id); break;
            case AVAE_ACT_TANH: AVAE_LAUNCH((K_HEAD_F(AVAE_ACT_TANH)), grid, block, lds_bytes, s, args, stamps, launch_id); break;
            default: AVAE_LAUNCH((K_HEAD_F(AVAE_ACT_IDENTITY)), grid, block, lds_bytes, s, args, stamps, launch_id); break;
        }
    }
#undef K_HEAD_B
#undef K_HEAD_F
}
void launch_small_latb(int compute_dtype, int act, const LaunchArgs& args, int grid_x, int grid_y, int lds_bytes, DevState* st, hipStream_t s,
                       unsigned long long* stamps, int launch_id) {
    const dim3 grid(grid_x, grid_y), block(kThreads);
#define K_LATB_B(A) k_small_latb<__bf16, A>
#define K_LATB_F(A) k_small_latb<float, A>
    if (compute_dtype == AVAE_BF16) {
        switch (act) {
            case AVAE_ACT_RELU: AVAE_LAUNCH((K_LATB_B(AVAE_ACT_RELU)), grid, block, lds_bytes, s, args, st, stamps, launch_id); break;
            case AVAE_ACT_SOFTPLUS: AVAE_LAUNCH((K_LATB_B(AVAE_ACT_SOFTPLUS)), grid, block, lds_bytes, s, args, st, stamps, launch_id); break;
            case AVAE_ACT_SIGMOID: AVAE_LAUNCH((K_LATB_B(AVAE_ACT_SIGMOID)), grid, block, lds_bytes, s, args, st, stamps, launch_id); break;
            case AVAE_ACT_TANH: AVAE_LAUNCH((K_LATB_B(AVAE_ACT_TANH)), grid, block, lds_bytes, s, args, st, stamps, launch_id); break;
            default: AVAE_LAUNCH((K_LATB_B(AVAE_ACT_IDENTITY)), grid, block, lds_bytes, s, args, st, stamps, launch_id); break;
        }
    } else {
        switch (act) {
            case AVAE_ACT_RELU: AVAE_LAUNCH((K_LATB_F(AVAE_ACT_RELU)), grid, block, lds_bytes, s, args, st, stamps, launch_id); break;
            case AVAE_ACT_SOFTPLUS: AVAE_LAUNCH((K_LATB_F(AVAE_ACT_SOFTPLUS)), grid, block, lds_bytes, s, args, st, stamps, launch_id); break;
            case AVAE_ACT_SIGMOID: AVAE_LAUNCH((K_LATB_F(AVAE_ACT_SIGMOID)), grid, block, lds_bytes, s, args, st, stamps, launch_id); break;
            case AVAE_ACT_TANH: AVAE_LAUNCH((K_LATB_F(AVAE_ACT_TANH)), grid, block, lds_bytes, s, args, st, stamps, launch_id); break;
            default: AVAE_LAUNCH((K_LATB_F(AVAE_ACT_IDENTITY)), grid, block, lds_bytes, s, args, st, stamps, launch_id); break;
        }
    }
#undef K_LATB_B
#undef K_LATB_F
}

template <typename CT, bool ADAM>
__global__ void __launch_bounds__(kThreads) k_small_tn(const TnLaunchArgs args, unsigned long long* stamps, int launch_id) {
    constexpr int BM = 64, RING = 4, ES = (int)sizeof(CT), EPR = kTileBytesK / ES, NCH = 4;
    constexpr int kStage = 2 * BM * kTileBytesK;
    unsigned char* smem = avae_dyn_smem;
#ifdef AVAE_STAMPS
    unsigned long long sv[kStampWords] = {0, 0, 0, 0, 0, 0, 0, 0};
#endif
    AVAE_STAMP(0)
    const int part = blockIdx.x & 7, idx = blockIdx.x >> 3;
    int entry = blockIdx.y, t_piece = -1;
    if (args.xcd_pieces) {
        const TnPiece* row = args.pieces[part];
        int e = 0, lo = 0;
#pragma unroll
        for (int i = 0; i < kTnPieces; ++i) { const int ce = row[i].cum_end; if (idx >= ce) { e = i + 1; lo = ce; } }
        if (e >= kTnPieces) return;
        entry = row[e].item; t_piece = row[e].tile_off + idx - lo;
    }
    const TnItem w = args.items[entry];
    asm volatile("" :: "s"(w.A), "s"(w.B), "s"(w.out), "s"(w.lda), "s"(w.ldb), "s"(w.K), "s"(w.ld0), "s"(w.tile_off));
    float lr_t = 0.f;
    if constexpr (ADAM) lr_t = args.st->lr_t;
    int t;
    if (t_piece >= 0) {
        t = t_piece;
    } else {
        const int nt = w.tile_cnt;
        const int q = nt >> 3, r = nt & 7;
        if (idx >= q + (part < r ? 1 : 0)) return;
        t = (part < r ? part * (q + 1) : r * (q + 1) + (part - r) * q) + idx + w.tile_off;
    }
    const int tid = threadIdx.x, lane = tid & 63, wave = __builtin_amdgcn_readfirstlane(tid >> 6);
    const int wr = wave >> 1, wc = wave & 1, fr = lane & 15, fq = lane >> 4;
    const int tm = t / w.tiles_n, tn = t - tm * w.tiles_n;
    const int m0 = tm * BM, n0 = tn * BM;
    const int nk = (w.K * ES) / kTileBytesK;
    typedef const __attribute__((address_space(1))) void* gp_t;
    typedef __attribute__((address_space(3))) void* lp_t;
    const unsigned char* src[NCH];
    size_t kadv[NCH];
#pragma unroll
    for (int c = 0; c < NCH; ++c) {
        const int r = (c * 4 + wave) * 8 + (lane >> 3);
        const bool is_a = c < 2;
        const int rr = is_a ? r : r - BM, sub = rr / EPR, k = rr - sub * EPR;
        const int lc = (lane & 7) ^ tn_swz<CT>(k);
        const size_t ld_b = (size_t)(is_a ? w.lda : w.ldb) * ES;
        kadv[c] = (size_t)EPR * ld_b;
        src[c] = reinterpret_cast<const unsigned char*>(is_a ? w.A : w.B) + (size_t)(is_a ? m0 : n0) * ES + (size_t)k * ld_b + (size_t)sub * kTileBytesK + lc * 16;
    }
#define AVAE_T_DMA(kt, buf)                                                                                             \
    { _Pragma("unroll") for (int c = 0; c < NCH; ++c)                                                                   \
        __builtin_amdgcn_global_load_lds((gp_t)(src[c] + (size_t)(kt) * kadv[c]), (lp_t)(smem + (buf) * kStage + (c * 4 + wave) * 1024), 16, 0, 0); }
    int offA[2], offB[2];
#pragma unroll
    for (int i = 0; i < 2; ++i) { offA[i] = tn_frag_off<CT>(wr * 32 + i * 16, lane); offB[i] = BM * kTileBytesK + tn_frag_off<CT>(wc * 32 + i * 16, lane); }
    AVAE_STAMP(1)
    const int npro = nk < RING - 1 ? nk : RING - 1;
    for (int p = 0; p < npro; ++p) AVAE_T_DMA(p, p)
    const int c4 = (tid & 15) * 4;
    f32x4 pth[4], pmm[4], pvv[4];
    auto fetch_state = [&]() {
#pragma unroll
        for (int k = 0; k < 4; ++k) {
            const int grow = m0 + (tid >> 4) + 16 * k, gcol = n0 + c4;
            const bool ok = grow < w.M && gcol < w.N;
            const float* gp = w.out + (size_t)(ok ? grow : m0) * w.ld0 + (ok ? gcol : n0);
            pth[k] = *reinterpret_cast<const f32x4*>(gp + args.d_theta);
            pmm[k] = *reinterpret_cast<const f32x4*>(gp + args.d_m);
            pvv[k] = *reinterpret_cast<const f32x4*>(gp + args.d_v);
        }
    };
    f32x4 acc[2][2];
#pragma unroll
    for (int i = 0; i < 2; ++i)
#pragma unroll
        for (int j = 0; j < 2; ++j) acc[i][j] = f32x4{0.f, 0.f, 0.f, 0.f};
    int buf = 0;
    for (int kt = 0; kt < nk; ++kt) {
        const int rem = nk - 1 - kt;
        if (rem >= 2) asm volatile("s_waitcnt vmcnt(8)" ::: "memory");
        else if (rem == 1) asm volatile("s_waitcnt vmcnt(4)" ::: "memory");
        else asm volatile("s_waitcnt vmcnt(0)" ::: "memory");
        asm volatile("s_barrier" ::: "memory");
        if (kt == 0) { AVAE_STAMP(2) }
        const unsigned char* Sb = smem + buf * kStage;
        u32x4 a0[2], b0[2], a1[2], b1[2];
#pragma unroll
        for (int i = 0; i < 2; ++i) { a0[i] = tn_frag<CT>(Sb, offA[i], 0); b0[i] = tn_frag<CT>(Sb, offB[i], 0); }
        const int fill = buf == 0 ? RING - 1 : buf - 1;
        if (kt + RING - 1 < nk) AVAE_T_DMA(kt + RING - 1, fill)
#pragma unroll
        for (int i = 0; i < 2; ++i) { a1[i] = tn_frag<CT>(Sb, offA[i], 1); b1[i] = tn_frag<CT>(Sb, offB[i], 1); }
        if constexpr (sizeof(CT) == 2) { tn_wait_lds(); tn_frags_ready(a0); tn_frags_ready(b0); tn_frags_ready(a1); tn_frags_ready(b1); }
#pragma unroll
        for (int i = 0; i < 2; ++i)
#pragma unroll
            for (int j = 0; j < 2; ++j) mma<CT>(b0[j], a0[i], acc[i][j]);
#pragma unroll
        for (int i = 0; i < 2; ++i)
#pragma unroll
            for (int j = 0; j < 2; ++j) mma<CT>(b1[j], a1[i], acc[i][j]);
        buf = buf + 1 == RING ? 0 : buf + 1;
    }
#undef AVAE_T_DMA
    AVAE_STAMP(3)
    if constexpr (!ADAM) {
#pragma unroll
        for (int i = 0; i < 2; ++i) {
            const int row = m0 + wr * 32 + i * 16 + fr;
#pragma unroll
            for (int j = 0; j < 2; ++j) {
                const int col = n0 + wc * 32 + j * 16 + 4 * fq;
                if (row < w.M && col < w.N) {
                    const float g[4] = {acc[i][j][0], acc[i][j][1], acc[i][j][2], acc[i][j][3]};
                    store_row<float>(w.out + (size_t)row * w.ld0 + col, g, w.N - col);
                }
            }
        }
    } else {
        constexpr int LDT = 65;
        float* T = reinterpret_cast<float*>(smem);
        fetch_state();
        lds_barrier();
#pragma unroll
        for (int i = 0; i < 2; ++i)
#pragma unroll
            for (int j = 0; j < 2; ++j)
#pragma unroll
                for (int e = 0; e < 4; ++e) T[(wr * 32 + i * 16 + fr) * LDT + wc * 32 + j * 16 + 4 * fq + e] = acc[i][j][e];
        lds_barrier();
        const float omb1 = 1.0f - args.beta1, omb2 = 1.0f - args.beta2;
        const int r4 = (tid & 15) * 4;
        float g[4][4], th[4][4], m[4][4], v[4][4];
#pragma unroll
        for (int k = 0; k < 4; ++k) {
            const int r = (tid >> 4) + 16 * k;
#pragma unroll
            for (int e = 0; e < 4; ++e) { g[k][e] = T[r * LDT + c4 + e]; th[k][e] = pth[k][e]; m[k][e] = pmm[k][e]; v[k][e] = pvv[k][e]; }
#pragma unroll
            for (int e = 0; e < 4; ++e) adam_update(g[k][e], m[k][e], v[k][e], th[k][e], omb1, omb2, lr_t, args.eps);
#pragma unroll
            for (int e = 0; e < 4; ++e) T[r * LDT + c4 + e] = th[k][e];
        }
        const bool full = m0 + BM <= w.M && n0 + BM <= w.N;
        auto store_group = [&](int k, float* gp, CT* wp) {
            store4<float>(gp, g[k]);
            store4<float>(gp + args.d_theta, th[k]); store4<float>(gp + args.d_m, m[k]); store4<float>(gp + args.d_v, v[k]);
            store4<CT>(wp, th[k]);
        };
        if (full) {
#pragma unroll
            for (int k = 0; k < 4; ++k) {
                const int grow = m0 + (tid >> 4) + 16 * k, gcol = n0 + c4;
                store_group(k, w.out + (size_t)grow * w.ld0 + gcol, reinterpret_cast<CT*>(w.W) + (size_t)grow * w.ldw + gcol);
            }
        } else {
#pragma unroll
            for (int k = 0; k < 4; ++k) {
                const int grow = m0 + (tid >> 4) + 16 * k, gcol = n0 + c4;
                float* gp = w.out + (size_t)grow * w.ld0 + gcol;
                CT* wp = reinterpret_cast<CT*>(w.W) + (size_t)grow * w.ldw + gcol;
                const int nv = w.N - gcol;
                if (grow < w.M && nv >= 4) {
                    store_group(k, gp, wp);
                } else if (grow < w.M && nv > 0) {
#pragma unroll
                    for (int e = 0; e < 3; ++e) if (e < nv) {
                        gp[e] = g[k][e]; gp[args.d_theta + e] = th[k][e]; gp[args.d_m + e] = m[k][e]; gp[args.d_v + e] = v[k][e]; wp[e] = to_ct<CT>(th[k][e]);
                    }
                    asm volatile("; partial quad" ::: "memory");
                }
            }
        }
        lds_barrier();
#pragma unroll
        for (int k = 0; k < 4; ++k) {
            const int c = (tid >> 4) + 16 * k;
            const int gcol = n0 + c, grow = m0 + r4;
            float t[4];
#pragma unroll
            for (int e = 0; e < 4; ++e) t[e] = T[(r4 + e) * LDT + c];
            CT* tp = reinterpret_cast<CT*>(w.Wt) + (size_t)gcol * w.ldt + grow;
            if (full) store4<CT>(tp, t);
            else if (gcol < w.N && grow < w.M) store_row<CT>(tp, t, w.M - grow);
        }
    }
    AVAE_STAMP(4)
    AVAE_STAMP_FLUSH()
}
void launch_small_tn(int compute_dtype, const TnLaunchArgs& args, int grid_x, int grid_y, hipStream_t s, unsigned long long* stamps, int launch_id) {
    const dim3 grid(grid_x, grid_y), block(kThreads);
    const int lds_bytes = 4 * 2 * 64 * kTileBytesK;
    if (compute_dtype == AVAE_BF16) {
        if (args.adam) AVAE_LAUNCH((k_small_tn<__bf16, true>), grid, block, lds_bytes, s, args, stamps, launch_id);
        else AVAE_LAUNCH((k_small_tn<__bf16, false>), grid, block, lds_bytes, s, args, stamps, launch_id);
    } else {
        if (args.adam) AVAE_LAUNCH((k_small_tn<float, true>), grid, block, lds_bytes, s, args, stamps, launch_id);
        else AVAE_LAUNCH((k_small_tn<float, false>), grid, block, lds_bytes, s, args, stamps, launch_id);
    }
}

template <typename CT, int KIND>
static void launch_small_act(int act, const LaunchArgs& args, dim3 grid, int lds_bytes, hipStream_t s, unsigned long long* stamps, int launch_id) {
    const dim3 block(kThreads);
    switch (act) {
        case AVAE_ACT_RELU: AVAE_LAUNCH((k_small<CT, KIND, AVAE_ACT_RELU>), grid, block, lds_bytes, s, args, stamps, launch_id); break;
        case AVAE_ACT_SOFTPLUS: AVAE_LAUNCH((k_small<CT, KIND, AVAE_ACT_SOFTPLUS>), grid, block, lds_bytes, s, args, stamps, launch_id); break;
        case AVAE_ACT_SIGMOID: AVAE_LAUNCH((k_small<CT, KIND, AVAE_ACT_SIGMOID>), grid, block, lds_bytes, s, args, stamps, launch_id); break;
        case AVAE_ACT_TANH: AVAE_LAUNCH((k_small<CT, KIND, AVAE_ACT_TANH>), grid, block, lds_bytes, s, args, stamps, launch_id); break;
        default: AVAE_LAUNCH((k_small<CT, KIND, AVAE_ACT_IDENTITY>), grid, block, lds_bytes, s, args, stamps, launch_id); break;
    }
}
void launch_small(int compute_dtype, const LaunchArgs& args, int grid_x, int grid_y, int lds_bytes, hipStream_t s, unsigned long long* stamps, int launch_id) {
    const dim3 grid(grid_x, grid_y);
    const int kind = args.items[0].kind == K_DGRAD_HIDDEN ? 1 : 0, act = args.items[0].act;
    if (args.items[0].kind == K_FWD_OUT_STORE) {
        const dim3 block(kThreads);
        if (compute_dtype == AVAE_BF16) AVAE_LAUNCH((k_small<__bf16, 2, AVAE_ACT_IDENTITY>), grid, block, lds_bytes, s, args, stamps, launch_id);
        else AVAE_LAUNCH((k_small<float, 2, AVAE_ACT_IDENTITY>), grid, block, lds_bytes, s, args, stamps, launch_id);
        return;
    }
    if (compute_dtype == AVAE_BF16) { if (kind) launch_small_act<__bf16, 1>(act, args, grid, lds_bytes, s, stamps, launch_id); else launch_small_act<__bf16, 0>(act, args, grid, lds_bytes, s, stamps, launch_id); }
    else { if (kind) launch_small_act<float, 1>(act, args, grid, lds_bytes, s, stamps, launch_id); else launch_small_act<float, 0>(act, args, grid, lds_bytes, s, stamps, launch_id); }
}

template <typename CT, int ACT>
__global__ void __launch_bounds__(kThreads) k_chain2(const LaunchArgs args, unsigned* counters, unsigned* err) {
    constexpr int BM = 32, RING = 4, ES = (int)sizeof(CT);
    constexpr int kStage = 64 * kTileBytesK;
    unsigned char* smem = avae_dyn_smem;
    const int part = blockIdx.x & 7, idx = blockIdx.x >> 3, half = args.n_items >> 1;
    const WorkItem w1 = args.items[blockIdx.y], w2 = args.items[half + blockIdx.y];
    asm volatile("" :: "s"(w1.A), "s"(w1.B), "s"(w1.out0), "s"(w1.lda), "s"(w1.ldb), "s"(w1.K), "s"(w1.ld0), "s"(w2.B), "s"(w2.out0), "s"(w2.ldb), "s"(w2.K), "s"(w2.ld0));
    int t;
    {
        const int nt = w1.tiles_m * w1.tiles_n;
        const int q = nt >> 3, r = nt & 7;
        if (idx >= q + (part < r ? 1 : 0)) return;
        t = (part < r ? part * (q + 1) : r * (q + 1) + (part - r) * q) + idx;
    }
    const int tid = threadIdx.x, lane = tid & 63, wave = __builtin_amdgcn_readfirstlane(tid >> 6);
    const int wr = wave >> 1, wc = wave & 1, fr = lane & 15, fq = lane >> 4;
    const int tm = t / w1.tiles_n, tn = t - tm * w1.tiles_n;
    const int m0 = tm * BM, n0 = tn * 32;
    typedef const __attribute__((address_space(1))) void* gp_t;
    typedef __attribute__((address_space(3))) void* lp_t;
    const int prow = wave * 8 + (lane >> 3), lc = ((lane & 7) ^ ((prow >> 1) & 7)) * 16;
    const int sw0 = (fq ^ (fr >> 1)) * 16;
    const int aoff = (wr * 16 + fr) * kTileBytesK, boff = (32 + wc * 16 + fr) * kTileBytesK;
    const int orow = m0 + wr * 16 + fr, ocol = n0 + wc * 16 + 4 * fq;
    f32x4 acc;
#define AVAE_C_LOOP(W, AUX)                                                                                               \
    {                                                                                                                     \
        const unsigned char* srcA = reinterpret_cast<const unsigned char*>((W).A) + (size_t)(m0 + prow) * (W).lda * ES + lc;   \
        const unsigned char* srcB = reinterpret_cast<const unsigned char*>((W).B) + (size_t)(n0 + prow) * (W).ldb * ES + lc;   \
        const int nk = ((W).K * ES) / kTileBytesK;                                                                        \
        auto dma = [&](int kt, int buf) __attribute__((always_inline)) {                                                  \
            __builtin_amdgcn_global_load_lds((gp_t)(srcA + (size_t)kt * kTileBytesK), (lp_t)(smem + buf * kStage + wave * 1024), 16, 0, AUX);       \
            __builtin_amdgcn_global_load_lds((gp_t)(srcB + (size_t)kt * kTileBytesK), (lp_t)(smem + buf * kStage + (4 + wave) * 1024), 16, 0, 0); };  \
        const int npro = nk < RING - 1 ? nk : RING - 1;                                                                   \
        for (int p = 0; p < npro; ++p) dma(p, p);                                                                         \
        acc = f32x4{0.f, 0.f, 0.f, 0.f};                                                                                  \
        int buf = 0;                                                                                                      \
        for (int kt = 0; kt < nk; ++kt) {                                                                                 \
            const int rem = nk - 1 - kt;                                                                                  \
            if (rem >= 2) asm volatile("s_waitcnt vmcnt(4)" ::: "memory");                                                \
            else if (rem == 1) asm volatile("s_waitcnt vmcnt(2)" ::: "memory");                                           \
            else asm volatile("s_waitcnt vmcnt(0)" ::: "memory");                                                         \
            asm volatile("s_barrier" ::: "memory");                                                                       \
            const unsigned char* Sb = smem + buf * kStage;                                                                 \
            const u32x4 a0 = *reinterpret_cast<const u32x4*>(Sb + aoff + sw0), b0 = *reinterpret_cast<const u32x4*>(Sb + boff + sw0);   \
            const int fill = buf == 0 ? RING - 1 : buf - 1;                                                               \
            if (kt + RING - 1 < nk) dma(kt + RING - 1, fill);                                                             \
            const u32x4 a1 = *reinterpret_cast<const u32x4*>(Sb + aoff + (sw0 ^ 64)), b1 = *reinterpret_cast<const u32x4*>(Sb + boff + (sw0 ^ 64)); \
            mma<CT>(b0, a0, acc);                                                                                         \
            mma<CT>(b1, a1, acc);                                                                                         \
            buf = buf + 1 == RING ? 0 : buf + 1;                                                                          \
        }                                                                                                                 \
    }
    AVAE_C_LOOP(w1, 0)
    if (orow < w1.M && ocol < w1.N) {
        CT* dst = reinterpret_cast<CT*>(w1.out0) + (size_t)orow * w1.ld0 + ocol;
        float v[4];
#pragma unroll
        for (int e = 0; e < 4; ++e) v[e] = act_fwd_t<ACT>(acc[e]);
        if (w1.N - ocol >= 4) {
            if constexpr (ES == 2) {
                const unsigned long long pk = (unsigned long long)pack_bf16(v[0], v[1]) | ((unsigned long long)pack_bf16(v[2], v[3]) << 32);
                __hip_atomic_store(reinterpret_cast<unsigned long long*>(dst), pk, __ATOMIC_RELAXED, __HIP_MEMORY_SCOPE_AGENT);
            } else {
                __hip_atomic_store(reinterpret_cast<unsigned long long*>(dst), __builtin_bit_cast(unsigned long long, float2{v[0], v[1]}), __ATOMIC_RELAXED, __HIP_MEMORY_SCOPE_AGENT);
                __hip_atomic_store(reinterpret_cast<unsigned long long*>(dst) + 1, __builtin_bit_cast(unsigned long long, float2{v[2], v[3]}), __ATOMIC_RELAXED, __HIP_MEMORY_SCOPE_AGENT);
            }
        } else {
            for (int e = 0; e < w1.N - ocol; ++e) {
                if constexpr (ES == 2) __hip_atomic_store(reinterpret_cast<unsigned short*>(dst) + e, __builtin_bit_cast(unsigned short, to_ct<CT>(v[e])), __ATOMIC_RELAXED, __HIP_MEMORY_SCOPE_AGENT);
                else __hip_atomic_store(reinterpret_cast<float*>(dst) + e, v[e], __ATOMIC_RELAXED, __HIP_MEMORY_SCOPE_AGENT);
            }
        }
    }
    asm volatile("s_waitcnt vmcnt(0)" ::: "memory");
    __syncthreads();
    if (tid == 0) {
        unsigned* cnt = counters + blockIdx.y * 64 + tm;
        const unsigned n = (unsigned)w1.tiles_n;
        const unsigned old = __hip_atomic_fetch_add(cnt, 1u, __ATOMIC_RELAXED, __HIP_MEMORY_SCOPE_AGENT);
        const unsigned target = (old / n + 1u) * n;
        int spins = 0;
        while ((int)(__hip_atomic_load(cnt, __ATOMIC_RELAXED, __HIP_MEMORY_SCOPE_AGENT) - target) < 0) {
            __builtin_amdgcn_s_sleep(1);
            if (++spins > (1 << 22)) { __hip_atomic_fetch_or(err, 1u, __ATOMIC_RELAXED, __HIP_MEMORY_SCOPE_AGENT); break; }
        }
    }
    __syncthreads();
    AVAE_C_LOOP(w2, 16)
#undef AVAE_C_LOOP
    if (orow < w2.M && ocol < w2.N) {
        float v[4];
#pragma unroll
        for (int e = 0; e < 4; ++e) v[e] = act_fwd_t<ACT>(acc[e]);
        store_row<CT>(reinterpret_cast<CT*>(w2.out0) + (size_t)orow * w2.ld0 + ocol, v, w2.N - ocol);
    }
}
template <typename CT> static void launch_chain2_act(int act, const LaunchArgs& args, dim3 grid, int lds, unsigned* counters, unsigned* err, hipStream_t s) {
    const dim3 block(kThreads);
    switch (act) {
    case AVAE_ACT_RELU: AVAE_LAUNCH((k_chain2<CT, AVAE_ACT_RELU>), grid, block, lds, s, args, counters, err); break;
    case AVAE_ACT_SOFTPLUS: AVAE_LAUNCH((k_chain2<CT, AVAE_ACT_SOFTPLUS>), grid, block, lds, s, args, counters, err); break;
    case AVAE_ACT_SIGMOID: AVAE_LAUNCH((k_chain2<CT, AVAE_ACT_SIGMOID>), grid, block, lds, s, args, counters, err); break;
    case AVAE_ACT_TANH: AVAE_LAUNCH((k_chain2<CT, AVAE_ACT_TANH>), grid, block, lds, s, args, counters, err); break;
    default: AVAE_LAUNCH((k_chain2<CT, AVAE_ACT_IDENTITY>), grid, block, lds, s, args, counters, err); break;
    }
}
void launch_chain2(int compute_dtype, const LaunchArgs& args, int grid_x, int grid_y, int lds_bytes, unsigned* counters, unsigned* err, hipStream_t s) {
    const dim3 grid(grid_x, grid_y);
    if (compute_dtype == AVAE_BF16) launch_chain2_act<__bf16>(args.items[0].act, args, grid, lds_bytes, counters, err, s);
    else launch_chain2_act<float>(args.items[0].act, args, grid, lds_bytes, counters, err, s);
}

constexpr int kProducers = 4;

static void grouped_attrs_once() {
    static const bool once = [] {
        set_max_lds(k_grouped<__bf16, 64, 64, 4>); set_max_lds(k_grouped<__bf16, 128, 128, 2>); set_max_lds(k_grouped<__bf16, 256, 128, 3, 8, false, 0>);
        set_max_lds(k_grouped<float, 64, 64, 4>); set_max_lds(k_grouped<float, 128, 128, 2>); set_max_lds(k_grouped<float, 256, 128, 3, 8, false, 0>);
        set_max_lds(k_grouped<__bf16, 32, 64, 4>); set_max_lds(k_grouped<float, 32, 64, 4>);
        set_max_lds(k_grouped<__bf16, 64, 128, 4>); set_max_lds(k_grouped<float, 64, 128, 4>);
        set_max_lds(k_grouped<__bf16, 32, 32, 4>); set_max_lds(k_grouped<float, 32, 32, 4>);
        set_max_lds(k_grouped<__bf16, 256, 64, 3, 8, false, 0>); set_max_lds(k_grouped<float, 256, 64, 3, 8, false, 0>);
        set_max_lds(k_grouped<__bf16, 64, 64, 4, 4, true>); set_max_lds(k_grouped<__bf16, 128, 128, 2, 4, true>); set_max_lds(k_grouped<__bf16, 256, 128, 3, 8, true, kProducers>);
        set_max_lds(k_grouped<float, 64, 64, 4, 4, true>); set_max_lds(k_grouped<float, 128, 128, 2, 4, true>); set_max_lds(k_grouped<float, 256, 128, 3, 8, true, kProducers>);
        return true;
    }();
    (void)once;
}

#define AVAE_GO(CT, TNF)                                                                                                     \
    do {                                                                                                                     \
        if (tile_cfg == 0) AVAE_LAUNCH((k_grouped<CT, 64, 64, 4, 4, TNF>), grid, block, lds_bytes, s, args, st, lds_bytes, stamps, launch_id);        \
        else if (tile_cfg == 2) AVAE_LAUNCH((k_grouped<CT, 256, 128, 3, 8, TNF, (TNF ? kProducers : 0)>), grid, block, lds_bytes, s, args, st, lds_bytes, stamps, launch_id); \
        else AVAE_LAUNCH((k_grouped<CT, 128, 128, 2, 4, TNF>), grid, block, lds_bytes, s, args, st, lds_bytes, stamps, launch_id);                    \
    } while (0)

template <typename CT>
static void launch_grouped_masked(int tile_cfg, const LaunchArgs& args, dim3 grid, dim3 block, int lds_bytes, DevState* st, hipStream_t s,
                                  unsigned long long* stamps, int launch_id) {
    static const bool once = [] {
        set_max_lds(k_grouped<CT, 64, 64, 4, 4, false, 0, true>); set_max_lds(k_grouped<CT, 128, 128, 2, 4, false, 0, true>);
        set_max_lds(k_grouped<CT, 32, 64, 4, 4, false, 0, true>); set_max_lds(k_grouped<CT, 64, 128, 4, 4, false, 0, true>);
        set_max_lds(k_grouped<CT, 32, 32, 4, 4, false, 0, true>); set_max_lds(k_grouped<CT, 256, 64, 3, 8, false, 0, true>);
        return true;
    }();
    (void)once;
    if (tile_cfg == 6) AVAE_LAUNCH((k_grouped<CT, 256, 64, 3, 8, false, 0, true>), grid, block, lds_bytes, s, args, st, lds_bytes, stamps, launch_id);
    else if (tile_cfg == 3) AVAE_LAUNCH((k_grouped<CT, 32, 64, 4, 4, false, 0, true>), grid, block, lds_bytes, s, args, st, lds_bytes, stamps, launch_id);
    else if (tile_cfg == 5) AVAE_LAUNCH((k_grouped<CT, 32, 32, 4, 4, false, 0, true>), grid, block, lds_bytes, s, args, st, lds_bytes, stamps, launch_id);
// ... 1675 lines not shown
```

Before: 4.743 million.

## Replace by-value kernel args with precomputed per-tile descriptor tables and prefetch

Precomputes, for each small GEMM and TN+Adam launch, a table of 64-byte per-tile descriptors in device memory. Tiles are dealt across the XCDs, so each block loads one descriptor line instead of a multi-KB by-value argument struct and does no tile-index arithmetic. Each kernel also warms the next launch's descriptor lines through scalar loads, and a compiler flag preloads kernel arguments into registers. This adds a setup-time table build and an extra memory indirection per block, and the prefetch can be skipped via an env var.

```diff
diff --git a/__graft_entry__.py b/__graft_entry__.py
--- a/__graft_entry__.py
+++ b/__graft_entry__.py
@@ -8,7 +8,8 @@
 SOURCES = ["avae_kernels.hip", "avae_comm.hip", "avae_retrieve.hip", "avae_latent_stats.hip", "avae_aggpost.hip", "avae_gmm.hip", "avae_embed.hip", "avae_host.hip"]
 
 
-FLAGS = ["--offload-arch=gfx950", "-O3", "-std=c++17", "-fPIC", "-shared", "-Wno-unused-result"]
+FLAGS = ["--offload-arch=gfx950", "-O3", "-std=c++17", "-fPIC", "-shared", "-Wno-unused-result",
+         "-mllvm", "-amdgpu-kernarg-preload-count=5"]
 
 
 def _source_hash():
diff --git a/vae_assoc_amd/csrc/avae_device.h b/vae_assoc_amd/csrc/avae_device.h
--- a/vae_assoc_amd/csrc/avae_device.h
+++ b/vae_assoc_amd/csrc/avae_device.h
@@ -143,6 +143,35 @@
 };
 static_assert(sizeof(TnLaunchArgs) <= 4096, "kernel arguments are passed by value: 4 KiB");
 
+struct alignas(64) SmallDesc {
+    const unsigned char* a;
+    const unsigned char* b;
+    void* out;
+    const void* aux;
+    int lda, ldb, ld0, ldx;
+    int nk;
+    int mrem, nrem, xrem;
+};
+struct alignas(64) TnDesc {
+    const unsigned char* a;
+    const unsigned char* b;
+    float* out;
+    void* w;
+    void* wt;
+    int lda, ldb, ld0, ldw, ldt;
+    unsigned ext;
+    static constexpr unsigned pack(int nk, int mrem, int nrem) { return (unsigned)nk | (unsigned)(mrem < 64 ? mrem : 64) << 16 | (unsigned)(nrem < 64 ? nrem : 64) << 24; }
+};
+static_assert(sizeof(SmallDesc) == 64 && sizeof(TnDesc) == 64, "a descriptor is one cache line");
+struct DescWarm { const void* lines; int n; };
+struct TnDescArgs {
+    long long d_theta, d_m, d_v;
+    float beta1, beta2, eps;
+    const DevState* st;
+};
+constexpr int kTnDescHead = 8;
+static_assert(sizeof(TnDescArgs) <= 64, "a copy of the constants is one line of the table");
+
 struct DevState {
     long long step;
     float last_cost;
@@ -470,6 +499,9 @@
 void launch_small_tn(int compute_dtype, const TnLaunchArgs& args, int grid_x, int grid_y, hipStream_t s, unsigned long long* stamps, int launch_id);
 void launch_small_loss(int compute_dtype, const LaunchArgs& args, int grid_x, int grid_y, int lds_bytes, hipStream_t s, unsigned long long* stamps, int launch_id);
 void launch_small(int compute_dtype, const LaunchArgs& args, int grid_x, int grid_y, int lds_bytes, hipStream_t s, unsigned long long* stamps, int launch_id);
+void launch_small_desc(int compute_dtype, bool dgrad, int act, const SmallDesc* tab, int n_tiles, int lds_bytes, DescWarm warm, hipStream_t s,
+                       unsigned long long* stamps, int launch_id);
+void launch_small_tn_desc(int compute_dtype, const TnDesc* tab, int n_tiles, DescWarm warm, hipStream_t s, unsigned long long* stamps, int launch_id);
 void launch_reduce(const ReduceArgs& a, int n_blocks, hipStream_t s);
 void launch_chain2(int compute_dtype, const LaunchArgs& args, int grid_x, int grid_y, int lds_bytes, unsigned* counters, unsigned* err, hipStream_t s);
 
diff --git a/vae_assoc_amd/csrc/avae_host.hip b/vae_assoc_amd/csrc/avae_host.hip
--- a/vae_assoc_amd/csrc/avae_host.hip
+++ b/vae_assoc_amd/csrc/avae_host.hip
@@ -148,6 +148,8 @@
     bool tn = false;
     LaunchArgs args{};
     TnLaunchArgs targs{};
+    int desc_n = 0, desc_set = 0;
+    size_t desc_off = 0, desc_stride = 0;
     GatherArgs ga{};
     Col2imArgs ca{};
     ReduceArgs ra{};
@@ -260,6 +262,7 @@
     DevBuf agg_buf;
     DevBuf gmm_buf;
     DevBuf embed_buf;
+    DevBuf desc_buf;
     size_t off_chain = 0;
     size_t off_consts = 0, off_conv_tab = 0;
     std::vector<ConvA> conv_tab;
@@ -1908,11 +1911,137 @@
     }
     for (int i = 0; i < L.targs.n_items && L.type == 0; ++i) { TnItem& t = L.targs.items[i]; fix(t.A); fix(t.B); fix(t.out); }
     for (int i = 0; i < L.ga.n_seg && L.type == 1; ++i) fix(L.ga.seg[i].src);
+    L.desc_set = j;
     return L;
+}
+
+template <typename D> std::vector<D> deal_to_xcds(const std::vector<D> (&lists)[8]) {
+    size_t total = 0;
+    for (const auto& l : lists) total += l.size();
+    std::vector<D> out(total), spill;
+    std::vector<char> set(total, 0);
+    for (int p = 0; p < 8; ++p)
+        for (size_t i = 0; i < lists[p].size(); ++i) {
+            const size_t x = 8 * i + p;
+            if (x < total) { out[x] = lists[p][i]; set[x] = 1; } else spill.push_back(lists[p][i]);
+        }
+    size_t k = 0;
+    for (size_t x = 0; x < total; ++x) if (!set[x]) out[x] = spill[k++];
+    return out;
+}
+
+std::vector<SmallDesc> small_descs(const avae_handle* h, const Launch& L) {
+    std::vector<SmallDesc> lists[8];
+    const int es = h->es;
+    for (int y = 0; y < L.args.n_items; ++y) {
+        const WorkItem& w = L.args.items[y];
+        if (w.kind != L.args.items[0].kind || w.act != L.args.items[0].act || (w.kind != K_FWD_HIDDEN && w.kind != K_DGRAD_HIDDEN)) return {};
+        const int nt = w.tiles_m * w.tiles_n, q = nt >> 3, r = nt & 7;
+        for (int part = 0; part < 8; ++part)
+            for (int idx = 0; idx < q + (part < r ? 1 : 0); ++idx) {
+                const int t = (part < r ? part * (q + 1) : r * (q + 1) + (part - r) * q) + idx;
+                const int tm = t / w.tiles_n, tn = t - tm * w.tiles_n, m0 = tm * 32, n0 = tn * 32;
+                SmallDesc d{};
+                d.a = static_cast<const unsigned char*>(w.A) + (size_t)m0 * w.lda * es;
+                d.b = static_cast<const unsigned char*>(w.B) + (size_t)n0 * w.ldb * es;
+                d.out = static_cast<unsigned char*>(w.out0) + ((size_t)m0 * w.ld0 + n0) * es;
+                d.aux = w.kind == K_DGRAD_HIDDEN ? static_cast<const unsigned char*>(w.aux0) + ((size_t)m0 * w.ldx + n0) * es : nullptr;
+                d.lda = w.lda; d.ldb = w.ldb; d.ld0 = w.ld0; d.ldx = w.ldx;
+                d.nk = (w.K * es) / kTileBytesK;
+                d.mrem = w.M - m0; d.nrem = w.N - n0; d.xrem = w.ldx - n0;
+                lists[part].push_back(d);
+            }
+    }
+    return deal_to_xcds(lists);
+}
+
+std::vector<TnDesc> tn_descs(const avae_handle* h, const Launch& L) {
+    std::vector<TnDesc> lists[8];
+    const TnLaunchArgs& a = L.targs;
+    const int es = h->es;
+    for (int y = 0; y < L.grid_y; ++y)
+        for (int x = 0; x < L.grid_x; ++x) {
+            const int part = x & 7, idx = x >> 3;
+            int entry = y, t = -1;
+            if (a.xcd_pieces) {
+                int e = 0, lo = 0;
+                for (int i = 0; i < kTnPieces; ++i) { const int ce = a.pieces[part][i].cum_end; if (idx >= ce) { e = i + 1; lo = ce; } }
+                if (e >= kTnPieces) continue;
+                entry = a.pieces[part][e].item; t = a.pieces[part][e].tile_off + idx - lo;
+            } else {
+                if (entry >= a.n_items) continue;
+                const int nt = a.items[entry].tile_cnt, q = nt >> 3, r = nt & 7;
+                if (idx >= q + (part < r ? 1 : 0)) continue;
+                t = (part < r ? part * (q + 1) : r * (q + 1) + (part - r) * q) + idx + a.items[entry].tile_off;
+            }
+            const TnItem& w = a.items[entry];
+            const int tm = t / w.tiles_n, tn = t - tm * w.tiles_n, m0 = tm * 64, n0 = tn * 64;
+            const int nk = (w.K * es) / kTileBytesK;
+            if (nk > 65535 || !w.W || !w.Wt) return {};
+            TnDesc d{};
+            d.a = static_cast<const unsigned char*>(w.A) + (size_t)m0 * es;
+            d.b = static_cast<const unsigned char*>(w.B) + (size_t)n0 * es;
+            d.out = w.out + (size_t)m0 * w.ld0 + n0;
+            d.w = static_cast<unsigned char*>(w.W) + ((size_t)m0 * w.ldw + n0) * es;
+            d.wt = static_cast<unsigned char*>(w.Wt) + ((size_t)n0 * w.ldt + m0) * es;
+            d.lda = w.lda; d.ldb = w.ldb; d.ld0 = w.ld0; d.ldw = w.ldw; d.ldt = w.ldt;
+            d.ext = TnDesc::pack(nk, w.M - m0, w.N - n0);
+            lists[part].push_back(d);
+        }
+    return deal_to_xcds(lists);
+}
+
+void build_descriptors(avae_handle* h, hipStream_t s) {
+    if (std::getenv("AVAE_NO_DESC")) return;
+    std::vector<unsigned char> tab;
+    auto add = [&](Launch& L) {
+        if (L.type != 0 || !((L.cfg == 7 && !L.tn) || (L.cfg == 12 && L.tn && L.targs.adam))) return;
+        const size_t off = tab.size();
+        size_t stride = 0;
+        int n = 0;
+        for (int j = 0; j < kMultiSteps; ++j) {
+            const Launch Lj = j == 0 ? L : relocated(h, L, j);
+            const size_t at = tab.size();
+            if (L.tn) {
+                const std::vector<TnDesc> d = tn_descs(h, Lj);
+                if (d.empty()) { tab.resize(off); return; }
+                const TnDescArgs ca = {L.targs.d_theta, L.targs.d_m, L.targs.d_v, L.targs.beta1, L.targs.beta2, L.targs.eps, L.targs.st};
+                tab.resize(at + (kTnDescHead + d.size()) * 64, 0);
+                for (int p = 0; p < kTnDescHead; ++p) std::memcpy(tab.data() + at + 64 * p, &ca, sizeof(ca));
+                std::memcpy(tab.data() + at + 64 * kTnDescHead, d.data(), d.size() * 64);
+                n = (int)d.size();
+            } else {
+                const std::vector<SmallDesc> d = small_descs(h, Lj);
+                if (d.empty()) { tab.resize(off); return; }
+                tab.resize(at + d.size() * 64);
+                std::memcpy(tab.data() + at, d.data(), d.size() * 64);
+                n = (int)d.size();
+            }
+            stride = tab.size() - at;
+        }
+        L.desc_n = n; L.desc_off = off; L.desc_stride = stride;
+    };
+    for (Launch& L : h->plain.fwd) add(L);
+    for (Launch& L : h->bwd) add(L);
+    for (Launch& L : h->wgrad_adam) add(L);
+    if (tab.empty()) return;
+    HIP_OK(hipMemcpyAsync(h->desc_buf.ensure(tab.size()), tab.data(), tab.size(), hipMemcpyHostToDevice, s));
+    HIP_OK(hipStreamSynchronize(s));
+}
+
+template <typename D> const D* desc_of(const avae_handle* h, const Launch& L) {
+    return reinterpret_cast<const D*>(h->desc_buf.as<unsigned char>() + L.desc_off + (size_t)L.desc_set * L.desc_stride);
+}
+
+DescWarm warm_for(const avae_handle* h, const Launch* next, int next_set) {
+    if (!next || next->desc_n == 0 || next_set >= kMultiSteps) return DescWarm{nullptr, 0};
+    return DescWarm{h->desc_buf.as<unsigned char>() + next->desc_off + (size_t)next_set * next->desc_stride,
+                    next->desc_n + (next->tn ? kTnDescHead : 0)};
 }
 
 void dump_launch(const Launch& L) {
     std::fprintf(stderr, "[avae] launch %s type=%d cfg=%d items=%d blocks=%d\n", L.name.c_str(), L.type, L.cfg, L.count, L.blocks);
+    if (L.desc_n) std::fprintf(stderr, "        descriptors=%d set=%d\n", L.desc_n, L.desc_set);
     for (int i = 0; i < L.args.n_items && L.type == 0; ++i)
         std::fprintf(stderr, "        item kind=%d M=%d N=%d K=%d lda=%d ldb=%d tiles=%dx%d\n", L.args.items[i].kind, L.args.items[i].M,
                      L.args.items[i].N, L.args.items[i].K, L.args.items[i].lda, L.args.items[i].ldb, L.args.items[i].tiles_m, L.args.items[i].tiles_n);
@@ -1925,7 +2054,7 @@
                      L.ca.seg[i].g.OH, L.ca.seg[i].g.k, L.ca.seg[i].lddp, L.ca.seg[i].lda, (const void*)L.ca.seg[i].g0, L.ca.seg[i].tiles_r, L.ca.seg[i].tiles_c);
 }
 
-void run_launch(avae_handle* h, const Launch& L, hipStream_t s, unsigned long long* stamps, int stamp) {
+void run_launch(avae_handle* h, const Launch& L, hipStream_t s, unsigned long long* stamps, int stamp, DescWarm warm = DescWarm{nullptr, 0}) {
     Timed t(h, s, L.name);
     if (L.type == 1) launch_gather(h->cfg.compute_dtype, L.ga, L.blocks, s);
     else if (L.type == 2) launch_col2im(h->cfg.compute_dtype, L.ca, L.blocks, s);
@@ -1940,7 +2069,9 @@
     else if (L.cfg == 11) launch_small_head(h->cfg.compute_dtype, L.lean_act, L.args, L.grid_x, L.grid_y, L.lds, s, stamps, stamp);
     else if (L.cfg == 10) launch_small_latb(h->cfg.compute_dtype, L.lean_act, L.args, L.grid_x, L.grid_y, L.lds, h->state(), s, stamps, stamp);
     else if (L.cfg == 9) launch_small_loss(h->cfg.compute_dtype, L.args, L.grid_x, L.grid_y, L.lds, s, stamps, stamp);
+    else if (L.cfg == 7 && L.desc_n) launch_small_desc(h->cfg.compute_dtype, L.args.items[0].kind == K_DGRAD_HIDDEN, L.args.items[0].act, desc_of<SmallDesc>(h, L), L.desc_n, L.lds, warm, s, stamps, stamp);
     else if (L.cfg == 7) launch_small(h->cfg.compute_dtype, L.args, L.grid_x, L.grid_y, L.lds, s, stamps, stamp);
+    else if (L.tn && L.cfg == 12 && L.desc_n) launch_small_tn_desc(h->cfg.compute_dtype, desc_of<TnDesc>(h, L), L.desc_n, warm, s, stamps, stamp);
     else if (L.tn && L.cfg == 12) launch_small_tn(h->cfg.compute_dtype, L.targs, L.grid_x, L.grid_y, s, stamps, stamp);
     else if (L.tn) launch_grouped_tn(h->cfg.compute_dtype, L.cfg, L.targs, L.grid_x, L.grid_y, L.lds, h->state(), s, stamps, stamp);
     else launch_grouped(h->cfg.compute_dtype, L.cfg, L.args, L.grid_x, L.grid_y, L.lds, h->state(), s, stamps, stamp);
@@ -1958,7 +2089,8 @@
     return false;
 }
 
-void run_set(avae_handle* h, const std::vector<Launch>& ls, size_t lo, size_t hi, int j, hipStream_t s, int stamp_base = -1, bool train = false) {
+void run_set(avae_handle* h, const std::vector<Launch>& ls, size_t lo, size_t hi, int j, hipStream_t s, int stamp_base = -1, bool train = false,
+             const Launch* after = nullptr, int after_set = 0) {
     unsigned long long* stamps = nullptr;
 #ifdef AVAE_STAMPS
     if (stamp_base >= 0) stamps = h->at<unsigned long long>(h->off_stamps);
@@ -1971,8 +2103,10 @@
     }
     for (size_t i = lo; i < hi && i < ls.size(); ++i) {
         const int k = stamp_base + (int)(i - lo);
-        if (j == 0 && !(hyper && has_hyper_item(ls[i]))) run_launch(h, ls[i], s, stamps, k);
-        else run_launch(h, relocated(h, ls[i], j, hyper), s, stamps, k);
+        const bool last = i + 1 >= hi || i + 1 >= ls.size();
+        const DescWarm warm = last ? warm_for(h, after, after_set) : warm_for(h, &ls[i + 1], j);
+        if (j == 0 && !(hyper && has_hyper_item(ls[i]))) run_launch(h, ls[i], s, stamps, k, warm);
+        else run_launch(h, relocated(h, ls[i], j, hyper), s, stamps, k, warm);
     }
 }
 
@@ -2139,12 +2273,14 @@
     LAUNCH_OK("fill");
 }
 
-void step_body(avae_handle* h, const std::vector<Launch>& fwd, hipStream_t s, int j, int stamp_base = -1) {
+void step_body(avae_handle* h, const std::vector<Launch>& fwd, hipStream_t s, int j, int stamp_base = -1, bool more = false) {
     auto sb = [&](size_t k) { return stamp_base < 0 ? -1 : stamp_base + (int)k; };
-    run_set(h, fwd, 0, fwd.size(), j, s, stamp_base, true);
-    run_set(h, h->bwd, 0, h->bwd.size(), j, s, sb(fwd.size()), true);
-    if (!h->wgrad_adam.empty() && !h->clip_on && !h->ema_on) {
-        run_set(h, h->wgrad_adam, 0, h->wgrad_adam.size(), j, s, sb(fwd.size() + h->bwd.size()), true);
+    auto first_of = [](const std::vector<Launch>& ls) { return ls.empty() ? nullptr : &ls[0]; };
+    const bool fused = !h->wgrad_adam.empty() && !h->clip_on && !h->ema_on;
+    run_set(h, fwd, 0, fwd.size(), j, s, stamp_base, true, first_of(h->bwd), j);
+    run_set(h, h->bwd, 0, h->bwd.size(), j, s, sb(fwd.size()), true, fused ? first_of(h->wgrad_adam) : nullptr, j);
+    if (fused) {
+        run_set(h, h->wgrad_adam, 0, h->wgrad_adam.size(), j, s, sb(fwd.size() + h->bwd.size()), true, more ? first_of(fwd) : nullptr, j + 1);
         return;
     }
     run_set(h, h->wgrad, 0, h->wgrad.size(), j, s, sb(fwd.size() + h->bwd.size()), true);
@@ -2161,7 +2297,7 @@
         }, true);
         for (int gi = 0; gi < 2; ++gi) p.multi[gi] = capture(h, [&](hipStream_t cs) {
             run_prep_batch(h, x0.data(), nullptr, nullptr, h->B, kTrainSalt, cs, present, kMultiSizes[gi]);
-            for (int j = 0; j < kMultiSizes[gi]; ++j) step_body(h, p.fwd, cs, j);
+            for (int j = 0; j < kMultiSizes[gi]; ++j) step_body(h, p.fwd, cs, j, -1, j + 1 < kMultiSizes[gi]);
         }, true);
     } catch (...) { p.full.release(); p.multi[0].release(); p.multi[1].release(); throw; }
 }
@@ -2188,6 +2324,7 @@
         if (md.conv && md.cdec[3].dense_map) fill_ones(h, md.cdec[3].Y, s);
     }
     build_training_plan(h);
+    build_descriptors(h, s);
     HIP_OK(hipMemcpyAsync(h->at<void>(h->off_adam), h->adam_items.data(), h->adam_items.size() * sizeof(AdamItem), hipMemcpyHostToDevice, s));
     HIP_OK(hipMemcpyAsync(h->at<void>(h->off_adam_b), h->adam_items_b.data(), h->adam_items_b.size() * sizeof(AdamItem), hipMemcpyHostToDevice, s));
     {
diff --git a/vae_assoc_amd/csrc/avae_kernels.hip b/vae_assoc_amd/csrc/avae_kernels.hip
--- a/vae_assoc_amd/csrc/avae_kernels.hip
+++ b/vae_assoc_amd/csrc/avae_kernels.hip
@@ -1298,6 +1298,78 @@
     AVAE_STAMP_FLUSH()
 }
 
+__device__ __forceinline__ unsigned desc_warm(const void* lines, int n, int wave) {
+    typedef const __attribute__((address_space(4))) unsigned* cu_t;
+    const int i = (blockIdx.x & 7) + 8 * (4 * (blockIdx.x >> 3) + wave);
+    return i < n ? *(cu_t)((unsigned long long)lines + 64ull * (unsigned)i) : 0u;
+}
+
+template <typename CT, int KIND, int ACT>
+__global__ void __launch_bounds__(kThreads) k_small_desc(const SmallDesc* __restrict__ tab, unsigned long long* stamps, int launch_id,
+                                                         const void* warm_lines, int warm_n) {
+    constexpr int RING = 4, ES = (int)sizeof(CT);
+    constexpr int kStage = 64 * kTileBytesK;
+    unsigned char* smem = avae_dyn_smem;
+#ifdef AVAE_STAMPS
+    unsigned long long sv[kStampWords] = {0, 0, 0, 0, 0, 0, 0, 0};
+#endif
+    AVAE_STAMP(0)
+    const SmallDesc d = tab[blockIdx.x];
+    const int tid = threadIdx.x, lane = tid & 63, wave = __builtin_amdgcn_readfirstlane(tid >> 6);
+    const int wr = wave >> 1, wc = wave & 1, fr = lane & 15, fq = lane >> 4;
+    const int nk = d.nk;
+    typedef const __attribute__((address_space(1))) void* gp_t;
+    typedef __attribute__((address_space(3))) void* lp_t;
+    const int prow = wave * 8 + (lane >> 3), lc = ((lane & 7) ^ ((prow >> 1) & 7)) * 16;
+    const unsigned char* srcA = d.a + (size_t)prow * d.lda * ES + lc;
+    const unsigned char* srcB = d.b + (size_t)prow * d.ldb * ES + lc;
+    const int lrow = wr * 16 + fr, lcol = wc * 16 + 4 * fq;
+    typename Quad<CT>::raw yq;
+    if constexpr (KIND == 1)
+        yq = *reinterpret_cast<const typename Quad<CT>::raw*>(reinterpret_cast<const CT*>(d.aux) + (ptrdiff_t)min(lrow, d.mrem - 1) * d.ldx + min(lcol, d.xrem - 4));
+#define AVAE_S_DMA(kt, buf)                                                                                             \
+    { __builtin_amdgcn_global_load_lds((gp_t)(srcA + (size_t)(kt) * kTileBytesK), (lp_t)(smem + (buf) * kStage + wave * 1024), 16, 0, 0);          \
+      __builtin_amdgcn_global_load_lds((gp_t)(srcB + (size_t)(kt) * kTileBytesK), (lp_t)(smem + (buf) * kStage + (4 + wave) * 1024), 16, 0, 0); }
+    AVAE_STAMP(1)
+    const int npro = nk < RING - 1 ? nk : RING - 1;
+    for (int p = 0; p < npro; ++p) AVAE_S_DMA(p, p)
+    const unsigned warmed = desc_warm(warm_lines, warm_n, wave);
+    const int sw0 = (fq ^ (fr >> 1)) * 16;
+    const int aoff = (wr * 16 + fr) * kTileBytesK, boff = (32 + wc * 16 + fr) * kTileBytesK;
+    f32x4 acc = {0.f, 0.f, 0.f, 0.f};
+    int buf = 0;
+    for (int kt = 0; kt < nk; ++kt) {
+        const int rem = nk - 1 - kt;
+        if (rem >= 2) asm volatile("s_waitcnt vmcnt(4)" ::: "memory");
+        else if (rem == 1) asm volatile("s_waitcnt vmcnt(2)" ::: "memory");
+        else asm volatile("s_waitcnt vmcnt(0)" ::: "memory");
+        asm volatile("s_barrier" ::: "memory");
+        if (kt == 0) { AVAE_STAMP(2) }
+        const unsigned char* Sb = smem + buf * kStage;
+        const u32x4 a0 = *reinterpret_cast<const u32x4*>(Sb + aoff + sw0), b0 = *reinterpret_cast<const u32x4*>(Sb + boff + sw0);
+        const int fill = buf == 0 ? RING - 1 : buf - 1;
+        if (kt + RING - 1 < nk) AVAE_S_DMA(kt + RING - 1, fill)
+        const u32x4 a1 = *reinterpret_cast<const u32x4*>(Sb + aoff + (sw0 ^ 64)), b1 = *reinterpret_cast<const u32x4*>(Sb + boff + (sw0 ^ 64));
+        mma<CT>(b0, a0, acc);
+        mma<CT>(b1, a1, acc);
+        buf = buf + 1 == RING ? 0 : buf + 1;
+    }
+#undef AVAE_S_DMA
+    AVAE_STAMP(3)
+    if (lrow < d.mrem && lcol < d.nrem) {
+        float v[4];
+#pragma unroll
+        for (int e = 0; e < 4; ++e) {
+            if constexpr (KIND == 0) v[e] = act_fwd_t<ACT>(acc[e]);
+            else v[e] = acc[e] * act_bwd_t<ACT>(quad_elem<CT>(yq, e));
+        }
+        store_row<CT>(reinterpret_cast<CT*>(d.out) + (size_t)lrow * d.ld0 + lcol, v, d.nrem - lcol);
+    }
+    asm volatile("" :: "s"(warmed));
+    AVAE_STAMP(4)
+    AVAE_STAMP_FLUSH()
+}
+
 thread_local LaunchEvents t_launch_events = {nullptr, nullptr};
 
 #define AVAE_LAUNCH(kernel, grid, block, lds, stream, ...)                                                   \
@@ -1726,10 +1798,174 @@
 #undef K_LATB_F
 }
 
+#ifdef AVAE_STAMPS
+#define AVAE_SV sv
+#else
+#define AVAE_SV nullptr
+#endif
+template <typename CT, bool ADAM, typename F>
+__device__ __forceinline__ void small_tn_tile(const TnDesc& d, const TnDescArgs& ca, F&& behind_prologue, unsigned char* smem, unsigned long long* sv) {
+    constexpr int BM = 64, RING = 4, ES = (int)sizeof(CT), EPR = kTileBytesK / ES, NCH = 4;
+    constexpr int kStage = 2 * BM * kTileBytesK;
+    const int tid = threadIdx.x, lane = tid & 63, wave = __builtin_amdgcn_readfirstlane(tid >> 6);
+    const int wr = wave >> 1, wc = wave & 1, fr = lane & 15, fq = lane >> 4;
+    const int nk = d.ext & 0xFFFF, mrem = (d.ext >> 16) & 0xFF, nrem = d.ext >> 24;
+    typedef const __attribute__((address_space(1))) void* gp_t;
+    typedef __attribute__((address_space(3))) void* lp_t;
+    const unsigned char* src[NCH];
+    size_t kadv[NCH];
+#pragma unroll
+    for (int c = 0; c < NCH; ++c) {
+        const int r = (c * 4 + wave) * 8 + (lane >> 3);
+        const bool is_a = c < 2;
+        const int rr = is_a ? r : r - BM, sub = rr / EPR, k = rr - sub * EPR;
+        const int lc = (lane & 7) ^ tn_swz<CT>(k);
+        const size_t ld_b = (size_t)(is_a ? d.lda : d.ldb) * ES;
+        kadv[c] = (size_t)EPR * ld_b;
+        src[c] = (is_a ? d.a : d.b) + (size_t)k * ld_b + (size_t)sub * kTileBytesK + lc * 16;
+    }
+#define AVAE_T_DMA(kt, buf)                                                                                             \
+    { _Pragma("unroll") for (int c = 0; c < NCH; ++c)                                                                   \
+        __builtin_amdgcn_global_load_lds((gp_t)(src[c] + (size_t)(kt) * kadv[c]), (lp_t)(smem + (buf) * kStage + (c * 4 + wave) * 1024), 16, 0, 0); }
+    int offA[2], offB[2];
+#pragma unroll
+    for (int i = 0; i < 2; ++i) { offA[i] = tn_frag_off<CT>(wr * 32 + i * 16, lane); offB[i] = BM * kTileBytesK + tn_frag_off<CT>(wc * 32 + i * 16, lane); }
+    AVAE_STAMP(1)
+    const int npro = nk < RING - 1 ? nk : RING - 1;
+    for (int p = 0; p < npro; ++p) AVAE_T_DMA(p, p)
+    const float lr_t = behind_prologue();
+    const int c4 = (tid & 15) * 4;
+    f32x4 pth[4], pmm[4], pvv[4];
+    auto fetch_state = [&]() {
+#pragma unroll
+        for (int k = 0; k < 4; ++k) {
+            const int lrow = (tid >> 4) + 16 * k;
+            const bool ok = lrow < mrem && c4 < nrem;
+            const float* gp = d.out + (size_t)(ok ? lrow : 0) * d.ld0 + (ok ? c4 : 0);
+            pth[k] = *reinterpret_cast<const f32x4*>(gp + ca.d_theta);
+            pmm[k] = *reinterpret_cast<const f32x4*>(gp + ca.d_m);
+            pvv[k] = *reinterpret_cast<const f32x4*>(gp + ca.d_v);
+        }
+    };
+    f32x4 acc[2][2];
+#pragma unroll
+    for (int i = 0; i < 2; ++i)
+#pragma unroll
+        for (int j = 0; j < 2; ++j) acc[i][j] = f32x4{0.f, 0.f, 0.f, 0.f};
+    int buf = 0;
+    for (int kt = 0; kt < nk; ++kt) {
+        const int rem = nk - 1 - kt;
+        if (rem >= 2) asm volatile("s_waitcnt vmcnt(8)" ::: "memory");
+        else if (rem == 1) asm volatile("s_waitcnt vmcnt(4)" ::: "memory");
+        else asm volatile("s_waitcnt vmcnt(0)" ::: "memory");
+        asm volatile("s_barrier" ::: "memory");
+        if (kt == 0) { AVAE_STAMP(2) }
+        const unsigned char* Sb = smem + buf * kStage;
+        u32x4 a0[2], b0[2], a1[2], b1[2];
+#pragma unroll
+        for (int i = 0; i < 2; ++i) { a0[i] = tn_frag<CT>(Sb, offA[i], 0); b0[i] = tn_frag<CT>(Sb, offB[i], 0); }
+        const int fill = buf == 0 ? RING - 1 : buf - 1;
+        if (kt + RING - 1 < nk) AVAE_T_DMA(kt + RING - 1, fill)
+#pragma unroll
+        for (int i = 0; i < 2; ++i) { a1[i] = tn_frag<CT>(Sb, offA[i], 1); b1[i] = tn_frag<CT>(Sb, offB[i], 1); }
+        if constexpr (sizeof(CT) == 2) { tn_wait_lds(); tn_frags_ready(a0); tn_frags_ready(b0); tn_frags_ready(a1); tn_frags_ready(b1); }
+#pragma unroll
+        for (int i = 0; i < 2; ++i)
+#pragma unroll
+            for (int j = 0; j < 2; ++j) mma<CT>(b0[j], a0[i], acc[i][j]);
+#pragma unroll
+        for (int i = 0; i < 2; ++i)
+#pragma unroll
+            for (int j = 0; j < 2; ++j) mma<CT>(b1[j], a1[i], acc[i][j]);
+        buf = buf + 1 == RING ? 0 : buf + 1;
+    }
+#undef AVAE_T_DMA
+    AVAE_STAMP(3)
+    if constexpr (!ADAM) {
+#pragma unroll
+        for (int i = 0; i < 2; ++i) {
+            const int row = wr * 32 + i * 16 + fr;
+#pragma unroll
+            for (int j = 0; j < 2; ++j) {
+                const int col = wc * 32 + j * 16 + 4 * fq;
+                if (row < mrem && col < nrem) {
+                    const float g[4] = {acc[i][j][0], acc[i][j][1], acc[i][j][2], acc[i][j][3]};
+                    store_row<float>(d.out + (size_t)row * d.ld0 + col, g, nrem - col);
+                }
+            }
+        }
+    } else {
+        constexpr int LDT = 65;
+        float* T = reinterpret_cast<float*>(smem);
+        fetch_state();
+        lds_barrier();
+#pragma unroll
+        for (int i = 0; i < 2; ++i)
+#pragma unroll
+            for (int j = 0; j < 2; ++j)
+#pragma unroll
+                for (int e = 0; e < 4; ++e) T[(wr * 32 + i * 16 + fr) * LDT + wc * 32 + j * 16 + 4 * fq + e] = acc[i][j][e];
+        lds_barrier();
+        const float omb1 = 1.0f - ca.beta1, omb2 = 1.0f - ca.beta2;
+        const int r4 = (tid & 15) * 4;
+        float g[4][4], th[4][4], m[4][4], v[4][4];
+#pragma unroll
+        for (int k = 0; k < 4; ++k) {
+            const int r = (tid >> 4) + 16 * k;
+#pragma unroll
+            for (int e = 0; e < 4; ++e) { g[k][e] = T[r * LDT + c4 + e]; th[k][e] = pth[k][e]; m[k][e] = pmm[k][e]; v[k][e] = pvv[k][e]; }
+#pragma unroll
+            for (int e = 0; e < 4; ++e) adam_update(g[k][e], m[k][e], v[k][e], th[k][e], omb1, omb2, lr_t, ca.eps);
+#pragma unroll
+            for (int e = 0; e < 4; ++e) T[r * LDT + c4 + e] = th[k][e];
+        }
+        const bool full = mrem >= BM && nrem >= BM;
+        auto store_group = [&](int k, float* gp, CT* wp) {
+            store4<float>(gp, g[k]);
+            store4<float>(gp + ca.d_theta, th[k]); store4<float>(gp + ca.d_m, m[k]); store4<float>(gp + ca.d_v, v[k]);
+            store4<CT>(wp, th[k]);
+        };
+        if (full) {
+#pragma unroll
+            for (int k = 0; k < 4; ++k) {
+                const int lrow = (tid >> 4) + 16 * k;
+                store_group(k, d.out + (size_t)lrow * d.ld0 + c4, reinterpret_cast<CT*>(d.w) + (size_t)lrow * d.ldw + c4);
+            }
+        } else {
+#pragma unroll
+            for (int k = 0; k < 4; ++k) {
+                const int lrow = (tid >> 4) + 16 * k;
+                float* gp = d.out + (size_t)lrow * d.ld0 + c4;
+                CT* wp = reinterpret_cast<CT*>(d.w) + (size_t)lrow * d.ldw + c4;
+                const int nv = nrem - c4;
+                if (lrow < mrem && nv >= 4) {
+                    store_group(k, gp, wp);
+                } else if (lrow < mrem && nv > 0) {
+#pragma unroll
+                    for (int e = 0; e < 3; ++e) if (e < nv) {
+                        gp[e] = g[k][e]; gp[ca.d_theta + e] = th[k][e]; gp[ca.d_m + e] = m[k][e]; gp[ca.d_v + e] = v[k][e]; wp[e] = to_ct<CT>(th[k][e]);
+                    }
+                    asm volatile("; partial quad" ::: "memory");
+                }
+            }
+        }
+        lds_barrier();
+#pragma unroll
+        for (int k = 0; k < 4; ++k) {
+            const int cc = (tid >> 4) + 16 * k;
+            float t[4];
+#pragma unroll
+            for (int e = 0; e < 4; ++e) t[e] = T[(r4 + e) * LDT + cc];
+            CT* tp = reinterpret_cast<CT*>(d.wt) + (size_t)cc * d.ldt + r4;
+            if (full) store4<CT>(tp, t);
+            else if (cc < nrem && r4 < mrem) store_row<CT>(tp, t, mrem - r4);
+        }
+    }
+}
+
 template <typename CT, bool ADAM>
 __global__ void __launch_bounds__(kThreads) k_small_tn(const TnLaunchArgs args, unsigned long long* stamps, int launch_id) {
-    constexpr int BM = 64, RING = 4, ES = (int)sizeof(CT), EPR = kTileBytesK / ES, NCH = 4;
-    constexpr int kStage = 2 * BM * kTileBytesK;
+    constexpr int BM = 64, ES = (int)sizeof(CT);
     unsigned char* smem = avae_dyn_smem;
 #ifdef AVAE_STAMPS
     unsigned long long sv[kStampWords] = {0, 0, 0, 0, 0, 0, 0, 0};
@@ -1758,164 +1994,49 @@
         if (idx >= q + (part < r ? 1 : 0)) return;
         t = (part < r ? part * (q + 1) : r * (q + 1) + (part - r) * q) + idx + w.tile_off;
     }
-    const int tid = threadIdx.x, lane = tid & 63, wave = __builtin_amdgcn_readfirstlane(tid >> 6);
-    const int wr = wave >> 1, wc = wave & 1, fr = lane & 15, fq = lane >> 4;
     const int tm = t / w.tiles_n, tn = t - tm * w.tiles_n;
     const int m0 = tm * BM, n0 = tn * BM;
-    const int nk = (w.K * ES) / kTileBytesK;
-    typedef const __attribute__((address_space(1))) void* gp_t;
-    typedef __attribute__((address_space(3))) void* lp_t;
-    const unsigned char* src[NCH];
-    size_t kadv[NCH];
-#pragma unroll
-    for (int c = 0; c < NCH; ++c) {
-        const int r = (c * 4 + wave) * 8 + (lane >> 3);
-        const bool is_a = c < 2;
-        const int rr = is_a ? r : r - BM, sub = rr / EPR, k = rr - sub * EPR;
-        const int lc = (lane & 7) ^ tn_swz<CT>(k);
-        const size_t ld_b = (size_t)(is_a ? w.lda : w.ldb) * ES;
-        kadv[c] = (size_t)EPR * ld_b;
-        src[c] = reinterpret_cast<const unsigned char*>(is_a ? w.A : w.B) + (size_t)(is_a ? m0 : n0) * ES + (size_t)k * ld_b + (size_t)sub * kTileBytesK + lc * 16;
-    }
-#define AVAE_T_DMA(kt, buf)                                                                                             \
-    { _Pragma("unroll") for (int c = 0; c < NCH; ++c)                                                                   \
-        __builtin_amdgcn_global_load_lds((gp_t)(src[c] + (size_t)(kt) * kadv[c]), (lp_t)(smem + (buf) * kStage + (c * 4 + wave) * 1024), 16, 0, 0); }
-    int offA[2], offB[2];
-#pragma unroll
-    for (int i = 0; i < 2; ++i) { offA[i] = tn_frag_off<CT>(wr * 32 + i * 16, lane); offB[i] = BM * kTileBytesK + tn_frag_off<CT>(wc * 32 + i * 16, lane); }
-    AVAE_STAMP(1)
-    const int npro = nk < RING - 1 ? nk : RING - 1;
-    for (int p = 0; p < npro; ++p) AVAE_T_DMA(p, p)
-    const int c4 = (tid & 15) * 4;
-    f32x4 pth[4], pmm[4], pvv[4];
-    auto fetch_state = [&]() {
-#pragma unroll
-        for (int k = 0; k < 4; ++k) {
-            const int grow = m0 + (tid >> 4) + 16 * k, gcol = n0 + c4;
-            const bool ok = grow < w.M && gcol < w.N;
-            const float* gp = w.out + (size_t)(ok ? grow : m0) * w.ld0 + (ok ? gcol : n0);
-            pth[k] = *reinterpret_cast<const f32x4*>(gp + args.d_theta);
-            pmm[k] = *reinterpret_cast<const f32x4*>(gp + args.d_m);
-            pvv[k] = *reinterpret_cast<const f32x4*>(gp + args.d_v);
-        }
-    };
-    f32x4 acc[2][2];
-#pragma unroll
-    for (int i = 0; i < 2; ++i)
-#pragma unroll
-        for (int j = 0; j < 2; ++j) acc[i][j] = f32x4{0.f, 0.f, 0.f, 0.f};
-    int buf = 0;
-    for (int kt = 0; kt < nk; ++kt) {
-        const int rem = nk - 1 - kt;
-        if (rem >= 2) asm volatile("s_waitcnt vmcnt(8)" ::: "memory");
-        else if (rem == 1) asm volatile("s_waitcnt vmcnt(4)" ::: "memory");
-        else asm volatile("s_waitcnt vmcnt(0)" ::: "memory");
-        asm volatile("s_barrier" ::: "memory");
-        if (kt == 0) { AVAE_STAMP(2) }
-        const unsigned char* Sb = smem + buf * kStage;
-        u32x4 a0[2], b0[2], a1[2], b1[2];
-#pragma unroll
-        for (int i = 0; i < 2; ++i) { a0[i] = tn_frag<CT>(Sb, offA[i], 0); b0[i] = tn_frag<CT>(Sb, offB[i], 0); }
-        const int fill = buf == 0 ? RING - 1 : buf - 1;
-        if (kt + RING - 1 < nk) AVAE_T_DMA(kt + RING - 1, fill)
-#pragma unroll
-        for (int i = 0; i < 2; ++i) { a1[i] = tn_frag<CT>(Sb, offA[i], 1); b1[i] = tn_frag<CT>(Sb, offB[i], 1); }
-        if constexpr (sizeof(CT) == 2) { tn_wait_lds(); tn_frags_ready(a0); tn_frags_ready(b0); tn_frags_ready(a1); tn_frags_ready(b1); }
-#pragma unroll
-        for (int i = 0; i < 2; ++i)
-#pragma unroll
-            for (int j = 0; j < 2; ++j) mma<CT>(b0[j], a0[i], acc[i][j]);
-#pragma unroll
-        for (int i = 0; i < 2; ++i)
-#pragma unroll
-            for (int j = 0; j < 2; ++j) mma<CT>(b1[j], a1[i], acc[i][j]);
-        buf = buf + 1 == RING ? 0 : buf + 1;
-    }
-#undef AVAE_T_DMA
-    AVAE_STAMP(3)
-    if constexpr (!ADAM) {
-#pragma unroll
-        for (int i = 0; i < 2; ++i) {
-            const int row = m0 + wr * 32 + i * 16 + fr;
-#pragma unroll
-            for (int j = 0; j < 2; ++j) {
-                const int col = n0 + wc * 32 + j * 16 + 4 * fq;
-                if (row < w.M && col < w.N) {
-                    const float g[4] = {acc[i][j][0], acc[i][j][1], acc[i][j][2], acc[i][j][3]};
-                    store_row<float>(w.out + (size_t)row * w.ld0 + col, g, w.N - col);
-                }
-            }
-        }
-    } else {
-        constexpr int LDT = 65;
-        float* T = reinterpret_cast<float*>(smem);
-        fetch_state();
-        lds_barrier();
-#pragma unroll
-        for (int i = 0; i < 2; ++i)
-#pragma unroll
-            for (int j = 0; j < 2; ++j)
-#pragma unroll
-                for (int e = 0; e < 4; ++e) T[(wr * 32 + i * 16 + fr) * LDT + wc * 32 + j * 16 + 4 * fq + e] = acc[i][j][e];
-        lds_barrier();
-        const float omb1 = 1.0f - args.beta1, omb2 = 1.0f - args.beta2;
-        const int r4 = (tid & 15) * 4;
-        float g[4][4], th[4][4], m[4][4], v[4][4];
-#pragma unroll
-        for (int k = 0; k < 4; ++k) {
-            const int r = (tid >> 4) + 16 * k;
-#pragma unroll
-            for (int e = 0; e < 4; ++e) { g[k][e] = T[r * LDT + c4 + e]; th[k][e] = pth[k][e]; m[k][e] = pmm[k][e]; v[k][e] = pvv[k][e]; }
-#pragma unroll
-            for (int e = 0; e < 4; ++e) adam_update(g[k][e], m[k][e], v[k][e], th[k][e], omb1, omb2, lr_t, args.eps);
-#pragma unroll
-            for (int e = 0; e < 4; ++e) T[r * LDT + c4 + e] = th[k][e];
-        }
-        const bool full = m0 + BM <= w.M && n0 + BM <= w.N;
-        auto store_group = [&](int k, float* gp, CT* wp) {
-            store4<float>(gp, g[k]);
-            store4<float>(gp + args.d_theta, th[k]); store4<float>(gp + args.d_m, m[k]); store4<float>(gp + args.d_v, v[k]);
-            store4<CT>(wp, th[k]);
-        };
-        if (full) {
-#pragma unroll
-            for (int k = 0; k < 4; ++k) {
-                const int grow = m0 + (tid >> 4) + 16 * k, gcol = n0 + c4;
-                store_group(k, w.out + (size_t)grow * w.ld0 + gcol, reinterpret_cast<CT*>(w.W) + (size_t)grow * w.ldw + gcol);
-            }
-        } else {
-#pragma unroll
-            for (int k = 0; k < 4; ++k) {
-                const int grow = m0 + (tid >> 4) + 16 * k, gcol = n0 + c4;
-                float* gp = w.out + (size_t)grow * w.ld0 + gcol;
-                CT* wp = reinterpret_cast<CT*>(w.W) + (size_t)grow * w.ldw + gcol;
-                const int nv = w.N - gcol;
-                if (grow < w.M && nv >= 4) {
-                    store_group(k, gp, wp);
-                } else if (grow < w.M && nv > 0) {
-#pragma unroll
-                    for (int e = 0; e < 3; ++e) if (e < nv) {
-                        gp[e] = g[k][e]; gp[args.d_theta + e] = th[k][e]; gp[args.d_m + e] = m[k][e]; gp[args.d_v + e] = v[k][e]; wp[e] = to_ct<CT>(th[k][e]);
-                    }
-                    asm volatile("; partial quad" ::: "memory");
-                }
-            }
-        }
-        lds_barrier();
-#pragma unroll
-        for (int k = 0; k < 4; ++k) {
-            const int c = (tid >> 4) + 16 * k;
-            const int gcol = n0 + c, grow = m0 + r4;
-            float t[4];
-#pragma unroll
-            for (int e = 0; e < 4; ++e) t[e] = T[(r4 + e) * LDT + c];
-            CT* tp = reinterpret_cast<CT*>(w.Wt) + (size_t)gcol * w.ldt + grow;
-            if (full) store4<CT>(tp, t);
-            else if (gcol < w.N && grow < w.M) store_row<CT>(tp, t, w.M - grow);
-        }
-    }
+    TnDesc d;
+    d.a = reinterpret_cast<const unsigned char*>(w.A) + (size_t)m0 * ES;
+    d.b = reinterpret_cast<const unsigned char*>(w.B) + (size_t)n0 * ES;
+    d.out = w.out + (size_t)m0 * w.ld0 + n0;
+    d.w = reinterpret_cast<CT*>(w.W) + (size_t)m0 * w.ldw + n0;
+    d.wt = reinterpret_cast<CT*>(w.Wt) + (size_t)n0 * w.ldt + m0;
+    d.lda = w.lda; d.ldb = w.ldb; d.ld0 = w.ld0; d.ldw = w.ldw; d.ldt = w.ldt;
+    d.ext = TnDesc::pack((w.K * ES) / kTileBytesK, w.M - m0, w.N - n0);
+    const TnDescArgs ca = {args.d_theta, args.d_m, args.d_v, args.beta1, args.beta2, args.eps, args.st};
+    small_tn_tile<CT, ADAM>(d, ca, [lr_t]() { return lr_t; }, smem, AVAE_SV);
     AVAE_STAMP(4)
     AVAE_STAMP_FLUSH()
+}
+
+template <typename CT>
+__global__ void __launch_bounds__(kThreads) k_small_tn_desc(const TnDesc* __restrict__ tab, unsigned long long* stamps, int launch_id,
+                                                            const void* warm_lines, int warm_n) {
+    unsigned char* smem = avae_dyn_smem;
+#ifdef AVAE_STAMPS
+    unsigned long long sv[kStampWords] = {0, 0, 0, 0, 0, 0, 0, 0};
+#endif
+    AVAE_STAMP(0)
+    const TnDescArgs ca = *reinterpret_cast<const TnDescArgs*>(tab + (blockIdx.x & 7));
+    const TnDesc d = tab[kTnDescHead + blockIdx.x];
+    unsigned warmed = 0;
+    small_tn_tile<CT, true>(d, ca, [&]() {
+        typedef const __attribute__((address_space(4))) float* cf_t;
+        const int wave = __builtin_amdgcn_readfirstlane(threadIdx.x >> 6);
+        const float lr_t = *(cf_t)(unsigned long long)&ca.st->lr_t;
+        warmed = desc_warm(warm_lines, warm_n, wave);
+        return lr_t;
+    }, smem, AVAE_SV);
+    asm volatile("" :: "s"(warmed));
+    AVAE_STAMP(4)
+    AVAE_STAMP_FLUSH()
+}
+void launch_small_tn_desc(int compute_dtype, const TnDesc* tab, int n_tiles, DescWarm warm, hipStream_t s, unsigned long long* stamps, int launch_id) {
+    const dim3 grid(n_tiles), block(kThreads);
+    const int lds_bytes = 4 * 2 * 64 * kTileBytesK;
+    if (compute_dtype == AVAE_BF16) AVAE_LAUNCH((k_small_tn_desc<__bf16>), grid, block, lds_bytes, s, tab, stamps, launch_id, warm.lines, warm.n);
+    else AVAE_LAUNCH((k_small_tn_desc<float>), grid, block, lds_bytes, s, tab, stamps, launch_id, warm.lines, warm.n);
 }
 void launch_small_tn(int compute_dtype, const TnLaunchArgs& args, int grid_x, int grid_y, hipStream_t s, unsigned long long* stamps, int launch_id) {
     const dim3 grid(grid_x, grid_y), block(kThreads);
@@ -1951,6 +2072,24 @@
     }
     if (compute_dtype == AVAE_BF16) { if (kind) launch_small_act<__bf16, 1>(act, args, grid, lds_bytes, s, stamps, launch_id); else launch_small_act<__bf16, 0>(act, args, grid, lds_bytes, s, stamps, launch_id); }
     else { if (kind) launch_small_act<float, 1>(act, args, grid, lds_bytes, s, stamps, launch_id); else launch_small_act<float, 0>(act, args, grid, lds_bytes, s, stamps, launch_id); }
+}
+
+template <typename CT, int KIND>
+static void launch_small_desc_act(int act, const SmallDesc* tab, dim3 grid, int lds_bytes, DescWarm warm, hipStream_t s, unsigned long long* stamps, int launch_id) {
+    const dim3 block(kThreads);
+    switch (act) {
+        case AVAE_ACT_RELU: AVAE_LAUNCH((k_small_desc<CT, KIND, AVAE_ACT_RELU>), grid, block, lds_bytes, s, tab, stamps, launch_id, warm.lines, warm.n); break;
+        case AVAE_ACT_SOFTPLUS: AVAE_LAUNCH((k_small_desc<CT, KIND, AVAE_ACT_SOFTPLUS>), grid, block, lds_bytes, s, tab, stamps, launch_id, warm.lines, warm.n); break;
+        case AVAE_ACT_SIGMOID: AVAE_LAUNCH((k_small_desc<CT, KIND, AVAE_ACT_SIGMOID>), grid, block, lds_bytes, s, tab, stamps, launch_id, warm.lines, warm.n); break;
+        case AVAE_ACT_TANH: AVAE_LAUNCH((k_small_desc<CT, KIND, AVAE_ACT_TANH>), grid, block, lds_bytes, s, tab, stamps, launch_id, warm.lines, warm.n); break;
+        default: AVAE_LAUNCH((k_small_desc<CT, KIND, AVAE_ACT_IDENTITY>), grid, block, lds_bytes, s, tab, stamps, launch_id, warm.lines, warm.n); break;
+    }
+}
+void launch_small_desc(int compute_dtype, bool dgrad, int act, const SmallDesc* tab, int n_tiles, int lds_bytes, DescWarm warm, hipStream_t s,
+                       unsigned long long* stamps, int launch_id) {
+    const dim3 grid(n_tiles);
+    if (compute_dtype == AVAE_BF16) { if (dgrad) launch_small_desc_act<__bf16, 1>(act, tab, grid, lds_bytes, warm, s, stamps, launch_id); else launch_small_desc_act<__bf16, 0>(act, tab, grid, lds_bytes, warm, s, stamps, launch_id); }
+    else { if (dgrad) launch_small_desc_act<float, 1>(act, tab, grid, lds_bytes, warm, s, stamps, launch_id); else launch_small_desc_act<float, 0>(act, tab, grid, lds_bytes, warm, s, stamps, launch_id); }
 }
 
 template <typename CT, int ACT>
```

Measured after the change: 4.962 million, median of 6. +4.6%, better.
